# ArchDD/CPP-Raytracer-Rasterizer

Hardware: AMD Instinct MI355X
Metric: Mrays/s (primary+shadow) (higher is better)
Workload: dtype f32

## Files before the change

### cpp-raytracer-rasterizer_amd/capi/binned.cpp

```cpp
#include "capi.hpp"

namespace mirt {


int ensure_pairs(RtScratch &S, size_t cap)
{
    int r;
    if ((r = dev_realloc(&S.d_entries, cap)) || (r = dev_realloc(&S.d_pair_keys, cap)) || (r = dev_realloc(&S.d_pair_vals, cap)) ||
        (r = dev_realloc(&S.d_sorted_keys, cap)) || (r = dev_realloc(&S.d_tmp_vals, cap))) { S.cap_entries = 0; return r; }
    S.cap_entries = (uint32_t)cap;
    return MIRT_OK;
}

constexpr uint32_t BIN_MAX_KEYS = BUCKET_SORT_MAX_BUCKETS * 1024u - 1u;

void poll_pair_count(RtScratch &S)
{
    if (S.count_pending && hipEventQuery(S.ev_count) == hipSuccess) {
        S.known_pairs = *S.h_count; S.have_known = true; S.count_pending = false;
    }
    (void)hipGetLastError();
}

int bin_pass(RtScratch &S, BinSet bs, const OriginRow *cam_tab, const OriginRow *light_tab, uint32_t *counter, uint32_t *bin_off,
             bool fresh, uint32_t *npairs, bool may_guess = false)
{
    int rc;
    poll_pair_count(S);
    if (!fresh && may_guess && S.have_known && S.known_pairs > S.cap_used) fresh = true;
    const bool guess = fresh && may_guess && S.have_known;
    if (!S.d_entries || !S.cap_entries) {
        static const size_t initial = [] { const long v = env_int("MIRT_BIN_INITIAL_PAIRS", 0); return v > 0 ? (size_t)v : (size_t)1 << 20; }();
        if ((rc = ensure_pairs(S, initial))) return rc;
    }
    if (bs.nbins > BIN_MAX_KEYS) return fail(MIRT_ERR_INVALID_ARGUMENT, "binning: %u sort keys exceed the %u the bucket sort holds", bs.nbins, BIN_MAX_KEYS);
    bs.chunk_tris = 256;
    const dim3 bin_grid((unsigned)std::min<long long>((long long)((g.n + bs.chunk_tris - 1) / bs.chunk_tris) * bs.nframes, (long long)g.cu_count * 8));
    bs.counters = counter;
    const uint32_t nbuckets = bucket_sort_buckets(bs.nbins);
    if (nbuckets + 1 > S.cap_buckets) {
        S.cap_buckets = 0;
        if ((rc = dev_realloc(&S.d_bucket, (size_t)3 * (nbuckets + 1)))) return rc;
        HIP_TRY(hipMemsetAsync(S.d_bucket, 0, sizeof(uint32_t) * 3 * (nbuckets + 1), g.stream));
        S.cap_buckets = nbuckets + 1;
        S.bucket_dirty = false;
    }
    uint32_t *bcnt = S.d_bucket, *bbase = S.d_bucket + S.cap_buckets, *bcur = S.d_bucket + 2 * (size_t)S.cap_buckets;
    bs.bucket_cnt = bcnt; bs.nbuckets = nbuckets; bs.bucket_shift = bucket_sort_shift(bs.nbins);
    const size_t bin_lds = (size_t)nbuckets * sizeof(uint32_t);
    {
        static const bool once = [] {
            (void)hipFuncSetAttribute(reinterpret_cast<const void *>(&k_bin_pairs<512>), hipFuncAttributeMaxDynamicSharedMemorySize, 48 * 1024);
            (void)hipFuncSetAttribute(reinterpret_cast<const void *>(&k_bin_pairs<256>), hipFuncAttributeMaxDynamicSharedMemorySize, 48 * 1024);
            return true; }();
        (void)once;
    }
    static const int bin_wg_env = (int)env_int("MIRT_BIN_WG", 0);
    const int bin_wg = (bin_wg_env == 256 || bin_wg_env == 512) ? bin_wg_env : ((g.n < 400000 && g.in_flight >= 3) ? 256 : 512);
    if (guess) {
        const size_t want = (size_t)S.known_pairs + S.known_pairs / 2 + 4096;
        if (want > S.cap_entries) {
            HIP_TRY(hipStreamSynchronize(g.stream));
            if ((rc = ensure_pairs(S, want + want / 4))) return rc;
        }
    }
    bool publish_count = false;
    for (int attempt = 0; attempt < 2; attempt++) {
        static const uint32_t test_cap = [] { const long v = env_int("MIRT_TEST_PAIR_CAP", 0); return v > 0 ? (uint32_t)v : 0u; }();
        S.cap_used = (guess && test_cap && test_cap < S.cap_entries) ? test_cap : S.cap_entries;
        BinPairs pairs = { S.d_pair_keys, S.d_pair_vals, S.cap_used };
        bs.entries = S.d_entries; bs.cap_entries = S.cap_used;
        if (attempt) HIP_TRY(hipMemsetAsync(counter, 0, 4, g.stream));
        if (attempt || S.bucket_dirty) HIP_TRY(hipMemsetAsync(S.d_bucket, 0, sizeof(uint32_t) * 3 * (size_t)S.cap_buckets, g.stream));
        S.bucket_dirty = true;
        if (bin_wg == 256) hipLaunchKernelGGL(k_bin_pairs<256>, bin_grid, dim3(256), bin_lds, g.stream, g.d_tris, cam_tab, light_tab, g.n, bs, pairs);
        else hipLaunchKernelGGL(k_bin_pairs<512>, bin_grid, dim3(512), bin_lds, g.stream, g.d_tris, cam_tab, light_tab, g.n, bs, pairs);
        if (!fresh) break;
        if (guess) {
            if (!S.h_count) {
                HIP_TRY(hipHostMalloc(reinterpret_cast<void **>(&S.h_count), 64, hipHostMallocDefault));
                HIP_TRY(hipEventCreateWithFlags(&S.ev_count, hipEventDisableTiming));
            }
            if (!S.count_pending) publish_count = true;
            *npairs = S.known_pairs;
            break;
        }
        uint32_t total = 0;
        HIP_TRY(hipStreamSynchronize(g.stream));
        HIP_TRY(hipMemcpy(&total, counter, 4, hipMemcpyDeviceToHost));
        *npairs = total;
        S.known_pairs = total; S.have_known = true;
        S.count_pending = false;
        if (total <= S.cap_entries) break;
        if (attempt == 1) return fail(MIRT_ERR_HIP, "binning produced %u pairs twice with room for %u", total, S.cap_entries);
        if ((rc = ensure_pairs(S, (size_t)total + total / 8 + 4096))) return rc;
    }
#ifdef MIRT_BIN_STATS
    if (fresh) {
        uint32_t c[16];
        (void)hipMemcpy(c, counter, 64, hipMemcpyDeviceToHost);
        fprintf(stderr, "[mirt bin stats] flattened tests=%u max per work item=%u direct items=%u | huge: box valid=%u no box=%u (camera frame %u)\n", c[8], c[9], c[10], c[11], c[12], c[14]);
        fprintf(stderr, "[mirt bin stats] tris=%d frames=%d  pairs=%u  bins=%u | large items walked=%u level-1 rounds=%u level-2 steps=%u pairs=%u max steps/item=%u items>100 steps=%u\n",
                g.n, bs.nframes, *npairs, bs.nbins, c[2], c[3], c[4], c[5], c[6], c[7]);
        (void)hipMemset(counter + 2, 0, 56);
    }
#endif
    uint32_t *count_out = nullptr;
    if (publish_count) HIP_TRY(hipHostGetDevicePointer(reinterpret_cast<void **>(&count_out), S.h_count, 0));
    HIP_TRY(bucket_sort_pairs(S.d_pair_keys, S.d_pair_vals, counter, S.cap_used, *npairs, bs.nbins, S.d_sorted_keys, S.d_tmp_vals,
                              bcnt, bbase, bcur, bin_off, S.d_entries, g.cu_count, g.stream, count_out));
    S.bucket_dirty = false;
    if (publish_count) S.count_event_due = true;
    return MIRT_OK;
}

uint64_t light_key_of(const float *origins, int nlights)
{
    uint64_t key = 0xcbf29ce484222325ull ^ g.scene_version;
    auto mix = [&](const void *p, size_t nb) { const unsigned char *b = (const unsigned char *)p; for (size_t i = 0; i < nb; i++) { key ^= b[i]; key *= 0x100000001b3ull; } };
    mix(origins + 3, sizeof(float) * 3 * nlights); mix(&nlights, 4); mix(&g.n, 4);
    return key;
}

bool shell_range(const float *pos, double *dn, double *df)
{
    double n2 = 0.0, f2 = 0.0;
    for (int c = 0; c < 3; c++) {
        const double p = pos[c], lo = g.bbox_lo[c], hi = g.bbox_hi[c];
        const double near = p < lo ? lo - p : (p > hi ? p - hi : 0.0), far = std::max(std::fabs(p - lo), std::fabs(p - hi));
        n2 += near * near; f2 += far * far;
    }
    *dn = std::sqrt(n2); *df = std::sqrt(f2);
    return std::isfinite(*dn) && std::isfinite(*df) && *df > *dn;
}

void fill_light_frames(BinFrameDesc *frames, const RtFrame &f, int nlights, int cube_bins, int shells, uint32_t base_bins)
{
    memset(frames, 0, sizeof(BinFrameDesc) * 6 * nlights);
    for (int k = 0; k < nlights; k++) {
        double dn = 0.0, df = 0.0;
        const bool okr = shell_range(f.lpos[k], &dn, &df);
        for (int face = 0; face < 6; face++) {
            BinFrameDesc &d = frames[k * 6 + face];
            const int ax = face >> 1;
            d.P0[ax] = (face & 1) ? -1.0f : 1.0f;
            d.Pu[(ax + 1) % 3] = 1.0f;
            d.Pv[(ax + 2) % 3] = 1.0f;
            d.rw[ax] = d.P0[ax]; d.ru[(ax + 1) % 3] = 1.0f; d.rv[(ax + 2) % 3] = 1.0f;
            memcpy(d.S, f.lpos[k], 12);
            d.dmax = 2.0f;
            d.ulo = -1.0f; d.vlo = -1.0f; d.du = 2.0f / (float)cube_bins; d.dv = 2.0f / (float)cube_bins;
            d.pad_lo = -3.814697265625e-06f; d.pad_hi = 3.814697265625e-06f;
            d.nbu = cube_bins; d.nbv = cube_bins; d.j0 = 0; d.j1 = cube_bins;
            d.base = base_bins; d.tab = 1 + k;
            d.nshell = shells;
            d.shell_d0 = (float)dn;
            d.shell_iw = okr ? (float)(shells / (df - dn)) : 0.0f;
            base_bins += (uint32_t)(cube_bins * cube_bins);
        }
    }
}

int light_shells_for(int nlights, int cube_bins, uint32_t keys_in_front)
{
    static const int env = (int)env_int("MIRT_LIGHT_SHELLS", 0);
    const long long bins = 6ll * cube_bins * cube_bins * std::max(nlights, 1);
    int ns = (env >= 1 && env <= 64) ? env : 16;
    while (ns > 1 && bins * ns + keys_in_front + 64 > (long long)BIN_MAX_KEYS) ns >>= 1;
    return ns;
}

constexpr size_t LIGHT_COUNTER_BYTES = sizeof(uint32_t) * (128 + 6 * MIRT_MAX_LIGHTS);
int ensure_face_lists(RtScratch &S, int nlights)
{
    int rc;
    if (!S.d_bin_counters) {
        HIP_TRY(hipMalloc(reinterpret_cast<void **>(&S.d_bin_counters), LIGHT_COUNTER_BYTES));
        HIP_TRY(hipMemsetAsync(S.d_bin_counters, 0, LIGHT_COUNTER_BYTES, g.stream));
        S.d_face_counts = S.d_bin_counters + 128;
    }
    const size_t want = (size_t)6 * (size_t)nlights * (size_t)g.n;
    if (want > S.cap_face_sel) {
        HIP_TRY(hipStreamSynchronize(g.stream));
        S.cap_face_sel = 0;
        if ((rc = dev_realloc(&S.d_face_sel, want))) return rc;
        S.cap_face_sel = want;
    }
    return MIRT_OK;
}

int light_cache_ensure(RtScratch &S, const RtFrame &f, const float *origins, int nlights, int cube_bins)
{
    int rc;
    LightCache &C = g.lc;
    const uint64_t key = light_key_of(origins, nlights);
    if (C.valid && C.key == key && C.cube_bins == cube_bins) return MIRT_OK;
    C.valid = false;
    for (int o = 0; o < g.in_flight; o++)
        if (o != g.si) {
            HIP_TRY(hipEventRecord(g.streams[o].ev_order, g.streams[o].stream));
            HIP_TRY(hipStreamWaitEvent(g.stream, g.streams[o].ev_order, 0));
        }
    const int shells = light_shells_for(nlights, cube_bins, 0u);
    const uint32_t per_light = 6u * (uint32_t)(cube_bins * cube_bins) * (uint32_t)shells, nkeys = per_light * (uint32_t)nlights;
    if ((size_t)nlights * g.n > C.cap_tab) {
        C.cap_tab = 0;
        if ((rc = dev_realloc(&C.d_light_tab, (size_t)nlights * g.n))) return rc;
        C.cap_tab = (size_t)nlights * g.n;
    }
    if (nkeys + 1 > C.cap_bins) {
        C.cap_bins = 0;
        if ((rc = dev_realloc(&C.d_off, (size_t)nkeys + 1))) return rc;
        C.cap_bins = nkeys + 1;
    }
    if (!C.d_frames) HIP_TRY(hipMalloc(reinterpret_cast<void **>(&C.d_frames), sizeof(BinFrameDesc) * 6 * MIRT_MAX_LIGHTS));
    if (!C.d_origins) HIP_TRY(hipMalloc(reinterpret_cast<void **>(&C.d_origins), sizeof(float) * 3 * (1 + MIRT_MAX_LIGHTS)));
    if (!C.d_counter) { HIP_TRY(hipMalloc(reinterpret_cast<void **>(&C.d_counter), 512)); HIP_TRY(hipMemsetAsync(C.d_counter, 0, 512, g.stream)); }
    C.nbins = nkeys;
    C.nrows = 0;
    C.shells = shells;
    if (nlights > 0) {
        BinFrameDesc frames[6 * MIRT_MAX_LIGHTS];
        fill_light_frames(frames, f, nlights, cube_bins, shells, 0u);
        HIP_TRY(upload_small(C.d_frames, frames, sizeof(BinFrameDesc) * 6 * nlights, g.stream));
        HIP_TRY(upload_small(C.d_origins, origins, sizeof(float) * 3 * (1 + nlights), g.stream));
        if ((rc = ensure_face_lists(S, nlights))) return rc;
        HIP_TRY(hipMemsetAsync(S.d_face_counts, 0, sizeof(uint32_t) * 6 * nlights, g.stream));
        HIP_TRY(hipMemsetAsync(C.d_counter, 0, 512, g.stream));
        S.count_event_due = false;
        hipLaunchKernelGGL(k_select_faces, dim3((unsigned)std::min<long long>(((long long)g.n + 1023) / 1024, (long long)g.cu_count), nlights), dim3(1024), 0, g.stream,
                           g.d_tris, g.n, C.d_origins, C.d_frames, C.d_light_tab, S.d_face_sel, (uint32_t)g.n, S.d_face_counts);
        BinSet bs;
        memset(&bs, 0, sizeof bs);
        bs.frames = C.d_frames; bs.nframes = 6 * nlights; bs.nbins = nkeys; bs.bin_off = C.d_off;
        bs.face_lists = S.d_face_sel; bs.face_counts = S.d_face_counts; bs.face_stride = (uint32_t)g.n;
        uint32_t npairs = 0;
        if ((rc = bin_pass(S, bs, nullptr, C.d_light_tab, C.d_counter, C.d_off, true, &npairs))) return rc;
        S.count_event_due = false;
        if (npairs > C.cap_rows) {
            C.cap_rows = 0;
            if ((rc = dev_realloc(&C.d_rows, (size_t)npairs + npairs / 8 + 1024))) return rc;
            if ((rc = dev_realloc(&C.d_row_tri, (size_t)npairs + npairs / 8 + 1024))) return rc;
            C.cap_rows = npairs + npairs / 8 + 1024;
        }
        C.nrows = npairs;
        if (npairs)
            hipLaunchKernelGGL(k_expand_light_rows, dim3((unsigned)std::min<uint32_t>((npairs + 255) / 256, 4096u)), dim3(256), 0, g.stream,
                               C.d_off, S.d_entries, nlights, per_light, C.d_light_tab, g.n, C.d_rows, (const uint32_t *)nullptr, 0u, C.d_row_tri);
        HIP_TRY(hipGetLastError());
        S.bin_key_valid = false;
        S.last_bin_mode = -1;
    } else {
        HIP_TRY(hipMemsetAsync(C.d_off, 0, 4, g.stream));
    }
    if (g.in_flight > 1) {
        HIP_TRY(hipEventRecord(g.cur().ev_order, g.stream));
        for (int o = 0; o < g.in_flight; o++)
            if (o != g.si) HIP_TRY(hipStreamWaitEvent(g.streams[o].stream, g.cur().ev_order, 0));
    }
    C.key = key;
    C.cube_bins = cube_bins;
    C.valid = true;
    return MIRT_OK;
}

int camera_shells_for(long long tiles)
{
    static const int shells_env = (int)env_int("MIRT_CAM_SHELLS", 0);
    int ns = (int)std::min<long long>(8, std::max<long long>(1, (4ll << 20) / std::max<long long>(tiles, 1)));
    if (shells_env >= 1 && shells_env <= 64) ns = shells_env;
    while (ns > 1 && tiles * ns + 64 > (long long)BIN_MAX_KEYS) ns >>= 1;
    return ns;
}

bool frame_fits_binning(int W, int H)
{
    const long long tiles = (long long)((W + BIN_TILE - 1) / BIN_TILE) * ((H + BIN_TILE - 1) / BIN_TILE);
    return tiles + 64 <= (long long)BIN_MAX_KEYS;
}

constexpr int LIGHT_STABLE_FRAMES = 4;


int transient_light_pass(RtScratch &L, const RtFrame &f, const float *origins, int nlights, int cube_bins, int tshells, uint32_t per_light, uint64_t lkey, bool *kept,
                         unsigned long long *zero_hits )
{
    int rc;
    *kept = false;
    uint64_t key = 0xcbf29ce484222325ull ^ g.scene_version;
    {
        auto mix = [&](const void *p, size_t nb) { const unsigned char *b = (const unsigned char *)p; for (size_t i = 0; i < nb; i++) { key ^= b[i]; key *= 0x100000001b3ull; } };
        mix(&lkey, 8); mix(&cube_bins, 4); mix(&tshells, 4); mix(&g.n, 4); mix(&nlights, 4);
    }
    poll_pair_count(L);
    bool fresh = !L.bin_key_valid || L.bin_key != key;
    const bool may_guess = L.last_bin_mode == nlights;
    if (!fresh && L.have_known && L.known_pairs > L.cap_used) fresh = true;
    static const bool reuse_off = env_int("MIRT_BIN_REUSE", 1) == 0;
    if (!fresh && !reuse_off) { *kept = true; return MIRT_OK; }
    if ((rc = ensure_face_lists(L, nlights))) return rc;
    if (nlights > L.light_tab_lights || L.light_tab_n != g.n) {
        HIP_TRY(hipStreamSynchronize(g.stream));
        L.light_tab_lights = 0;
        if ((rc = dev_realloc(&L.d_light_tab, (size_t)nlights * g.n))) return rc;
        L.light_tab_lights = nlights;
        L.light_tab_n = g.n;
    }
    const uint32_t nkeys = per_light * (uint32_t)nlights;
    if (nkeys + 1 > L.cap_bins) {
        HIP_TRY(hipStreamSynchronize(g.stream));
        L.cap_bins = 0;
        if ((rc = dev_realloc(&L.d_bin_off, (size_t)nkeys + 1))) return rc;
        L.cap_bins = nkeys + 1;
    }
    if (!L.d_frames) HIP_TRY(hipMalloc(reinterpret_cast<void **>(&L.d_frames), sizeof(BinFrameDesc) * (6 * MIRT_MAX_LIGHTS) + sizeof(float) * 3 * (1 + MIRT_MAX_LIGHTS)));
    struct { BinFrameDesc frames[6 * MIRT_MAX_LIGHTS]; float origins[3 * (1 + MIRT_MAX_LIGHTS)]; } up;
    static_assert(sizeof(BinFrameDesc) % 4 == 0, "descriptors are uploaded as words");
    fill_light_frames(up.frames, f, nlights, cube_bins, tshells, 0u);
    float *d_origins = reinterpret_cast<float *>(L.d_frames + 6 * nlights);
    memcpy(reinterpret_cast<char *>(up.frames + 6 * nlights), origins, sizeof(float) * 3 * (1 + nlights));
    const ZeroJob zj = { L.d_bin_counters, (int)(LIGHT_COUNTER_BYTES / 4), reinterpret_cast<uint32_t *>(zero_hits), zero_hits ? 2 * HIT_SHARDS * HIT_SHARD_STRIDE : 0 };
    HIP_TRY(upload_small(L.d_frames, &up, sizeof(BinFrameDesc) * 6 * nlights + sizeof(float) * 3 * (1 + nlights), g.stream, &zj));
    hipLaunchKernelGGL(k_select_faces, dim3((unsigned)std::min<long long>(((long long)g.n + 1023) / 1024, (long long)g.cu_count), nlights), dim3(1024), 0, g.stream,
                       g.d_tris, g.n, d_origins, L.d_frames, L.d_light_tab, L.d_face_sel, (uint32_t)g.n, L.d_face_counts);
    BinSet bs;
    memset(&bs, 0, sizeof bs);
    bs.frames = L.d_frames; bs.nframes = 6 * nlights; bs.nbins = nkeys; bs.bin_off = L.d_bin_off;
    bs.face_lists = L.d_face_sel; bs.face_counts = L.d_face_counts; bs.face_stride = (uint32_t)g.n;
    if ((rc = bin_pass(L, bs, nullptr, L.d_light_tab, L.d_bin_counters, L.d_bin_off, true, &L.bin_entries, may_guess))) return rc;
    L.last_bin_mode = nlights;
    L.bin_key = key;
    L.bin_key_valid = true;
    if (L.cap_light_rows < L.cap_entries) {
        HIP_TRY(hipStreamSynchronize(g.stream));
        L.cap_light_rows = 0;
        if ((rc = dev_realloc(&L.d_light_rows, (size_t)L.cap_entries))) return rc;
        L.cap_light_rows = L.cap_entries;
    }
    const uint32_t expect = std::max<uint32_t>(L.bin_entries, 1u);
    hipLaunchKernelGGL(k_expand_light_rows, dim3((unsigned)std::min<uint32_t>((expect + 255) / 256, 4096u)), dim3(256), 0, g.stream,
                       L.d_bin_off, L.d_entries, nlights, per_light, L.d_light_tab, g.n, L.d_light_rows, L.d_bin_counters, L.cap_used, (uint32_t *)nullptr);
    return MIRT_OK;
}

int binned_pass(const RtFrame &f, const mirt_view *view, RtScratch &S, RtScratch &L, const float *origins, int nlights, int y0, int y1, BinnedPass *bp)
{
    int rc;
    g.stats.mode_used = MIRT_RT_BINNED;
    g.stats_sel_count = nullptr;
    static const int cube_override = (int)env_int("MIRT_CUBE_BINS", 0);
    int fine_bins = g.n < 2000 ? CUBE_BINS_MIN : (g.n < 20000 ? 2 * CUBE_BINS_MIN : 4 * CUBE_BINS_MIN);
    const bool fixed_grid = cube_override == 64 || cube_override == 128 || cube_override == 256;
    if (fixed_grid) fine_bins = cube_override;
    while (fine_bins > CUBE_BINS_MIN && 6ll * fine_bins * fine_bins * nlights * 4 > (long long)BIN_MAX_KEYS) fine_bins /= 2;

    const uint64_t lkey = light_key_of(origins, nlights);
    if (g.lc.track_key == lkey) g.lc.stable++;
    else { g.lc.track_key = lkey; g.lc.stable = 0; }
    const bool cached = g.lc.valid && g.lc.key == lkey && g.lc.cube_bins == fine_bins;
    const bool transient = nlights > 0 && !fixed_grid && !cached && g.lc.stable < LIGHT_STABLE_FRAMES;

    k_begin(MIRT_K_BIN);
    if (!transient && (rc = light_cache_ensure(L, f, origins, nlights, fine_bins))) return rc;
    const int cube_bins = transient ? CUBE_BINS_MIN : fine_bins;

    BinSet bs;
    memset(&bs, 0, sizeof bs);
    bs.frame0 = make_camera_frame(view, y0, y1, g.aa);
    bs.frames = nullptr; bs.nframes = 1;
    const int band_tile_rows = bs.frame0.j1 - bs.frame0.j0;
    const uint32_t key_shift_tiles = (uint32_t)bs.frame0.j0 * (uint32_t)bs.frame0.nbu;
    bs.frame0.base = 0u - key_shift_tiles;
    {
        const int ns = camera_shells_for((long long)bs.frame0.nbu * band_tile_rows);
        double dn = 0.0, df = 0.0;
        const bool okr = shell_range(view->pos, &dn, &df);
        bs.frame0.nshell = okr ? ns : 1;
        bs.frame0.shell_d0 = (float)dn;
        bs.frame0.shell_iw = okr ? (float)(ns / (df - dn)) : 0.0f;
    }
    const uint32_t cam_keys = (uint32_t)bs.frame0.nbu * (uint32_t)band_tile_rows * (uint32_t)bs.frame0.nshell;
    const int tshells = transient ? light_shells_for(nlights, cube_bins, 0u) : 1;
    const uint32_t per_light = 6u * (uint32_t)(cube_bins * cube_bins) * (uint32_t)tshells;
    bs.nbins = cam_keys;
    if (bs.nbins + 1 > S.cap_bins) {
        const size_t cap = (size_t)bs.nbins + 1;
        HIP_TRY(hipStreamSynchronize(g.stream));
        if ((rc = dev_realloc(&S.d_bin_off, cap))) { S.cap_bins = 0; return rc; }
        S.cap_bins = (uint32_t)cap;
        S.bin_key_valid = false;
    }
    if (!S.d_bin_counters) { HIP_TRY(hipMalloc(reinterpret_cast<void **>(&S.d_bin_counters), 512)); HIP_TRY(hipMemsetAsync(S.d_bin_counters, 0, 512, g.stream)); }
    if (S.sel_n != g.n) {
        HIP_TRY(hipStreamSynchronize(g.stream));
        S.sel_n = 0;
        if ((rc = dev_realloc(&S.d_sel, (size_t)g.n))) return rc;
        S.sel_n = g.n;
        S.bin_key_valid = false;
    }
    bs.bin_off = S.d_bin_off;

    uint64_t key = 0xcbf29ce484222325ull ^ g.scene_version;
    {
        auto mix = [&](const void *p, size_t nb) { const unsigned char *b = (const unsigned char *)p; for (size_t i = 0; i < nb; i++) { key ^= b[i]; key *= 0x100000001b3ull; } };
        mix(view, sizeof *view); mix(&y0, 4); mix(&y1, 4); mix(&g.n, 4); mix(&g.aa, 4);
    }
    const int bin_mode = 0;
    StreamState &ss = g.cur();
    ss.hits_clean[ss.hits_tog] = false;
    if (!S.d_frames) HIP_TRY(hipMalloc(reinterpret_cast<void **>(&S.d_frames), sizeof(BinFrameDesc) * (1 + 6 * MIRT_MAX_LIGHTS)));
    poll_pair_count(S);
    bool fresh = !S.bin_key_valid || S.bin_key != key;
    const bool may_guess = S.last_bin_mode == bin_mode;
    if (!fresh && S.have_known && S.known_pairs > S.cap_used) fresh = true;
    static const bool reuse_off = env_int("MIRT_BIN_REUSE", 1) == 0;
    const bool reuse = !fresh && !reuse_off;
    const uint32_t pairs_x = (uint32_t)((bs.frame0.nbu + 1) / 2);
    uint32_t group_rows[ORDER_GROUPS] = { 0 };
    for (int j = bs.frame0.j0; j < bs.frame0.j1; j++) group_rows[((uint32_t)j >> ORDER_STRIPE_SHIFT) & (ORDER_GROUPS - 1)]++;
    const uint32_t order_seg = pairs_x * *std::max_element(group_rows, group_rows + ORDER_GROUPS);
    const uint32_t *cam_off = S.d_bin_off - (size_t)key_shift_tiles * (size_t)bs.frame0.nshell;
    bool lights_kept = false, forked = false;
    if (transient) {
        static const bool side_off = env_int("MIRT_LIGHT_SIDE_STREAM", 1) == 0;
        hipStream_t main_stream = g.stream;
        forked = !reuse && !side_off;
        if (forked) {
            HIP_TRY(hipEventRecord(ss.ev_fork, main_stream));
            HIP_TRY(hipStreamWaitEvent(ss.aux, ss.ev_fork, 0));
            g.stream = ss.aux;
        }
        rc = transient_light_pass(L, f, origins, nlights, cube_bins, tshells, per_light, lkey, &lights_kept, reuse ? g.d_hits : nullptr);
        g.stream = main_stream;
        if (rc) return rc;
        if (forked) HIP_TRY(hipEventRecord(ss.ev_join, ss.aux));
    }
    if (reuse) {
        if (!(transient && !lights_kept)) HIP_TRY(hipMemsetAsync(g.d_hits, 0, HIT_BYTES, g.stream));
        g.stats.bins_reused = 1;
    } else {
        S.sel_parity ^= 1;
        SelectOut so;
        memset(&so, 0, sizeof so);
        so.cam_tab = S.d_cam_tab; so.sel = S.d_sel;
        so.sel_count = S.d_bin_counters + SEL_COUNT0 + S.sel_parity; so.sel_count_next = S.d_bin_counters + SEL_COUNT0 + (S.sel_parity ^ 1);
        so.zero_hits = g.d_hits; so.zero_counter = S.d_bin_counters;
        if ((rc = hist_prepare(S, bs.frame0, &so))) return rc;
        const unsigned sel_grid = (unsigned)std::min<long long>(((long long)g.n + 1023) / 1024, (long long)g.cu_count);
        hipLaunchKernelGGL(k_prep_select, dim3(sel_grid), dim3(1024), 0, g.stream, g.d_tris, g.n, bs.frame0, so);
        if ((rc = hist_publish(S))) return rc;
        bs.sel = S.d_sel; bs.sel_count = so.sel_count;
        g.stats_sel_count = so.sel_count;
        if ((rc = bin_pass(S, bs, S.d_cam_tab, nullptr, S.d_bin_counters, S.d_bin_off, true, &S.bin_entries, may_guess))) return rc;
        S.last_bin_mode = bin_mode;
        S.bin_key = key;
        S.bin_key_valid = true;
        if ((size_t)order_seg > S.cap_order) {
            HIP_TRY(hipStreamSynchronize(g.stream));
            S.cap_order = 0;
            if ((rc = dev_realloc(&S.d_order, (size_t)ORDER_GROUPS * ORDER_CLASSES * order_seg))) return rc;
            S.cap_order = order_seg;
        }
        hipLaunchKernelGGL(k_tile_order, dim3((pairs_x + 63) / 64, (unsigned)(bs.frame0.j1 - bs.frame0.j0)), dim3(64), 0, g.stream, cam_off, bs.frame0.nshell,
                           bs.frame0.nbu, bs.frame0.j0, bs.frame0.j1, S.d_bin_counters, S.cap_used, S.d_order, order_seg);
    }
    if (forked) HIP_TRY(hipStreamWaitEvent(g.stream, ss.ev_join, 0));
    k_end(MIRT_K_BIN);

    bp->cam_off = cam_off;
    bp->tiles_x = bs.frame0.nbu;
    bp->cam_shells = bs.frame0.nshell;
    bp->order_seg = order_seg;
    bp->transient = transient;
    bp->cube_bins = cube_bins;
    bp->light_shells = transient ? tshells : g.lc.shells;
    return MIRT_OK;
}

int hist_only_pass(const mirt_view *view)
{
    int rc;
    g.stream = g.cur().stream;
    RtScratch &S = g.cur().rt;
    if (S.cam_tab_n != g.n) {
        S.cam_tab_n = 0;
        if ((rc = dev_realloc(&S.d_cam_tab, (size_t)g.n))) return rc;
        S.cam_tab_n = g.n;
    }
    if (S.sel_n != g.n) {
        HIP_TRY(hipStreamSynchronize(g.stream));
        S.sel_n = 0;
        if ((rc = dev_realloc(&S.d_sel, (size_t)g.n))) return rc;
        S.sel_n = g.n;
    }
    if (!S.d_bin_counters) { HIP_TRY(hipMalloc(reinterpret_cast<void **>(&S.d_bin_counters), 512)); HIP_TRY(hipMemsetAsync(S.d_bin_counters, 0, 512, g.stream)); }
    S.bin_key_valid = false;
    const BinFrameDesc fr = make_camera_frame(view, 0, 0, g.aa);
    SelectOut so;
    memset(&so, 0, sizeof so);
    so.cam_tab = S.d_cam_tab; so.sel = S.d_sel;
    so.sel_count = S.d_bin_counters + HIST_SEL_COUNT; so.sel_count_next = S.d_bin_counters + HIST_SEL_COUNT + 1;
    if ((rc = hist_prepare(S, fr, &so))) return rc;
    if (!g.hist_armed) return MIRT_OK;
    HIP_TRY(hipMemsetAsync(so.sel_count, 0, 4, g.stream));
    const unsigned sel_grid = (unsigned)std::min<long long>(((long long)g.n + 1023) / 1024, (long long)g.cu_count);
    if (sel_grid) hipLaunchKernelGGL(k_prep_select, dim3(sel_grid), dim3(1024), 0, g.stream, g.d_tris, g.n, fr, so);
    HIP_TRY(hipGetLastError());
    return hist_publish(S);
}

int binned_trace(const RtFrame &f, RtScratch &S, RtScratch &L, const BinnedPass &bp)
{
    const bool transient = bp.transient;
    RtTraceFrame tf;
    memset(&tf, 0, sizeof tf);
    tf.f = f;
    tf.f.cam_tab = S.d_cam_tab;
    tf.f.light_tab = transient ? L.d_light_tab : g.lc.d_light_tab;
    tf.f.unsafe = nullptr;
    tf.cam_off = bp.cam_off;
    tf.cam_entries = S.d_entries;
    tf.sel = S.d_sel; tf.sel_count = S.d_bin_counters + SEL_COUNT0 + S.sel_parity;
    static const int lazy_env = (int)env_int("MIRT_LAZY_GEO", -1);
    tf.lazy_geo = lazy_env >= 0 ? (lazy_env != 0) : (g.n >= 400000);
    tf.geo = g.d_geo;
    tf.shade = g.d_shade;
    tf.light_off = transient ? L.d_bin_off : g.lc.d_off;
    tf.light_rows = transient ? L.d_light_rows : g.lc.d_rows;
    tf.light_tri = transient ? L.d_entries : g.lc.d_row_tri;
    tf.light_frames = transient ? L.d_frames : g.lc.d_frames;
    tf.tiles_x = bp.tiles_x;
    tf.cube_bins = bp.cube_bins;
    tf.cam_shells = bp.cam_shells;
    tf.light_shells = bp.light_shells;
    tf.pair_count = S.d_bin_counters;
    tf.pair_cap = S.cap_used;
    tf.light_pair_count = transient ? L.d_bin_counters : nullptr;
    tf.light_pair_cap = L.cap_used;
    tf.order = S.d_order; tf.order_count = S.d_bin_counters + 16; tf.order_seg = bp.order_seg;
    const dim3 tgrid(ORDER_GROUPS * bp.order_seg);
    const size_t lds = rt_trace_lds_bytes(1);
    k_begin(MIRT_K_TRACE);
    g.pending_counted = g.profiling;
    if (f.aa > 1) {
        if (g.profiling) hipLaunchKernelGGL((k_rt_trace2<true, true>), tgrid, dim3(64), lds, g.stream, tf);
        else hipLaunchKernelGGL((k_rt_trace2<true, false>), tgrid, dim3(64), lds, g.stream, tf);
    } else {
        static const int waves5_env = (int)env_int("MIRT_TR_WAVES5", -1);
        const bool waves5 = waves5_env >= 0 ? (waves5_env != 0) : (g.n >= 400000 || g.in_flight <= 2);
        if (g.profiling) hipLaunchKernelGGL((k_rt_trace2<false, true>), tgrid, dim3(64), lds, g.stream, tf);
        else if (waves5) hipLaunchKernelGGL((k_rt_trace2<false, false, 5>), tgrid, dim3(64), lds, g.stream, tf);
        else hipLaunchKernelGGL((k_rt_trace2<false, false>), tgrid, dim3(64), lds, g.stream, tf);
    }
    k_end(MIRT_K_TRACE);
    HIP_TRY(hipGetLastError());
    for (RtScratch *P : { &S, &L })
        if (P->count_event_due) {
            P->count_event_due = false;
            HIP_TRY(hipEventRecord(P->ev_count, g.stream));
            P->count_pending = true;
        }
    return MIRT_OK;
}

}
```

### cpp-raytracer-rasterizer_amd/capi/capi.hpp

```cpp
#pragma once

#include "../csrc/bin_sort.hpp"
#include "../csrc/comm.hpp"
#include "../csrc/cull.hpp"
#include "../csrc/dof.hpp"
#include "../csrc/rt_common.hpp"
#include "../csrc/raster_common.hpp"
#include "../csrc/rt_binned.hpp"
#include "../csrc/scan.hpp"
#include "env.hpp"

#include <cstdarg>
#include <cstdio>
#include <cstdlib>
#include <cstring>
#include <algorithm>
#include <cmath>
#include <vector>

#define MIRT_KERNEL __attribute__((global))

namespace mirt {

MIRT_KERNEL void k_prep_origin(const float *, int, const float *, v3, int, OriginRow *, OriginRow *, uint32_t *, unsigned long long *, uint32_t *);
template <int P> MIRT_KERNEL void k_rt_brute(const RtFrame);
template <int P> MIRT_KERNEL void k_rt_small(const RtFrame, int);
MIRT_KERNEL void k_rt_wave(const RtFrame);
struct RtTileFrame {
    RtFrame f;
    BinFrameDesc cam;
    int tiles_x, tiles_y;
    unsigned long long *clear_hits;
    float4 *tables;
};
MIRT_KERNEL void k_tile_tables(const RtTileFrame);
template <int TW, bool AA> MIRT_KERNEL void k_rt_tile2(const RtTileFrame);
template <int WG> MIRT_KERNEL void k_bin_pairs(const float *, const OriginRow *, const OriginRow *, int, BinSet, BinPairs);
struct TilePairRec { uint32_t tile, beg, nA, nB; };
constexpr int ORDER_CLASSES = 8, ORDER_GROUPS = 8;
struct RtTraceFrame {
    RtFrame f;
    const uint32_t *cam_off;
    const uint32_t *cam_entries;
    const GeoRow *geo;
    const ShadeRow *shade;
    const uint32_t *light_off;
    const LightRow *light_rows;
    const uint32_t *light_tri;
    const BinFrameDesc *light_frames;
    int tiles_x;
    int cube_bins;
    int cam_shells;
    int light_shells;
    const uint32_t *pair_count;
    uint32_t pair_cap;
    const TilePairRec *order;
    const uint32_t *order_count;
    uint32_t order_seg;
    const uint32_t *sel;
    const uint32_t *sel_count;
    int lazy_geo;
    const uint32_t *light_pair_count;
    uint32_t light_pair_cap;
};
template <bool AA, bool STATS, int WAVES = 4> MIRT_KERNEL void k_rt_trace2(const RtTraceFrame);
MIRT_KERNEL void k_prep_select(const float *, int, const BinFrameDesc, const SelectOut);
MIRT_KERNEL void k_select_faces(const float *, int, const float *, const BinFrameDesc *, OriginRow *, uint32_t *, uint32_t, uint32_t *);
MIRT_KERNEL void k_tile_order(const uint32_t *, int, int, int, int, uint32_t *, uint32_t, TilePairRec *, uint32_t);
MIRT_KERNEL void k_geo_table(const float *, int, GeoRow *, ShadeRow *);
MIRT_KERNEL void k_expand_light_rows(const uint32_t *, const uint32_t *, int, uint32_t, const OriginRow *, int, LightRow *, const uint32_t *, uint32_t, uint32_t *);
MIRT_KERNEL void k_cull(const float *, int, const CullParams, uint8_t *);
size_t rt_trace_lds_bytes(int waves);
int launch_raster(RasterFrame &f, RasterScratch &s, uint64_t scene_version, hipStream_t stream, hipEvent_t *ev, bool *ev_used);

extern char g_err[512];
int fail(int code, const char *fmt, ...);

#define HIP_TRY(expr)                                                                          \
    do {                                                                                       \
        hipError_t e_ = (expr);                                                                \
        if (e_ != hipSuccess)                                                                  \
            return fail(MIRT_ERR_HIP, "%s failed: %s (%s:%d)", #expr, hipGetErrorString(e_), __FILE__, __LINE__); \
    } while (0)

enum { EV_CALL0 = 0, EV_CALL1 = 1, EV_K0 = 2, EV_COUNT = 2 + 2 * 8 };
constexpr int MAX_FLIGHT = 4;
constexpr int SEL_COUNT0 = 80;
constexpr int HIST_SEL_COUNT = 82;
constexpr int HIST_RING = 4;
constexpr int HIST_SLOTS = HIST_RING + 1;
constexpr size_t HIT_BYTES = sizeof(unsigned long long) * HIT_SHARDS * HIT_SHARD_STRIDE;

struct RtScratch {
    OriginRow *d_cam_tab = nullptr;
    OriginRow *d_light_tab = nullptr;
    int cam_tab_n = 0, light_tab_n = 0, light_tab_lights = 0;
    float *d_origins = nullptr;
    uint32_t *d_flags = nullptr;
    BinFrameDesc *d_frames = nullptr;
    uint32_t *d_bin_off = nullptr, *d_bin_counters = nullptr;
    uint32_t *d_entries = nullptr;
    uint32_t *d_pair_keys = nullptr, *d_pair_vals = nullptr, *d_sorted_keys = nullptr;
    uint32_t *d_tmp_vals = nullptr;
    uint32_t *d_bucket = nullptr;
    uint32_t cap_buckets = 0;
    bool bucket_dirty = false;
    uint32_t *h_count = nullptr;
    hipEvent_t ev_count = nullptr;
    bool count_pending = false;
    bool count_event_due = false;
    bool have_known = false;
    uint32_t known_pairs = 0;
    uint32_t cap_bins = 0, cap_entries = 0;
    uint32_t cap_used = 0;
    uint64_t bin_key = 0;
    uint32_t bin_entries = 0;
    bool bin_key_valid = false;
    LightRow *d_light_rows = nullptr;
    uint32_t cap_light_rows = 0;
    TilePairRec *d_order = nullptr;
    uint32_t cap_order = 0;
    int last_bin_mode = -1;
    uint32_t *d_sel = nullptr;
    int sel_n = 0;
    int sel_parity = 0;
    uint32_t *d_face_sel = nullptr;
    size_t cap_face_sel = 0;
    uint32_t *d_face_counts = nullptr;
    uint32_t *d_hist = nullptr;
    uint32_t *h_hist = nullptr;
    hipEvent_t ev_hist[HIST_SLOTS] = {};
    uint64_t hist_key[HIST_SLOTS] = {};
    uint64_t hist_seq[HIST_SLOTS] = {};
    int hist_rows[HIST_SLOTS] = {}, hist_shift[HIST_SLOTS] = {};
    int hist_next = 0;

    void forget_scene() { bin_key_valid = false; have_known = false; count_pending = false; }
    void release();
};

struct LightCache {
    bool valid = false;
    uint64_t key = 0;
    int cube_bins = 0;
    uint64_t track_key = 0;
    int stable = 0;
    OriginRow *d_light_tab = nullptr;
    size_t cap_tab = 0;
    BinFrameDesc *d_frames = nullptr;
    uint32_t *d_off = nullptr;
    uint32_t cap_bins = 0, nbins = 0;
    LightRow *d_rows = nullptr;
    uint32_t *d_row_tri = nullptr;
    uint32_t cap_rows = 0, nrows = 0;
    int shells = 1;
    float *d_origins = nullptr;
    uint32_t *d_counter = nullptr;

    void release();
};

struct DofPlanes {
    float *rgb = nullptr, *fd = nullptr;
    uint32_t *xrgb = nullptr;
    int32_t *index = nullptr;
    float *zinv = nullptr;
    size_t cap_px = 0;

    int ensure(size_t px);
    void release();
};

struct StreamState {
    hipStream_t stream = nullptr;
    hipEvent_t ev_order = nullptr;
    hipStream_t aux = nullptr;
    hipEvent_t ev_fork = nullptr, ev_join = nullptr;
    hipEvent_t ev[EV_COUNT] = {};
    bool ev_used[8] = {};
    bool call_timed = false;
    RtScratch rt;
    RtScratch rt_lt;
    unsigned long long *d_hits[2] = {};
    bool hits_clean[2] = {};
    int hits_tog = 0;
    float4 *d_tile_tab = nullptr;
    DofPlanes dof;
    void *d_async = nullptr;
    RasterScratch raster;
    uint64_t culled_ver = 0;
    hipEvent_t ev_cull_read = nullptr;
    uint32_t cull_read_src = 0;

    int create();
    void release();
};

struct Ctx {
    bool init = false;
    bool profiling = false;
    int device = -1;
    int cu_count = 256;
    StreamState streams[MAX_FLIGHT];
    hipStream_t stream = nullptr;
    int in_flight = 1;
    uint64_t frame_no = 0;
    int si = 0;
    int ev_cur = 0;
    StreamState &cur() { return streams[si]; }

    int n = 0;
    float *d_tris = nullptr;
    uint8_t *d_culled = nullptr;
    int culled_latest = 0;
    uint64_t cull_calls = 0;
    GeoRow *d_geo = nullptr;
    ShadeRow *d_shade = nullptr;
    float bbox_lo[3] = { 0, 0, 0 }, bbox_hi[3] = { 0, 0, 0 };
    LightCache lc;
    unsigned long long *d_hits = nullptr;
    bool scene_finite = true;
    uint64_t scene_version = 0;
    uint64_t cull_version = 0;
    int soft_samples = 1;
    int aa = 1;
    int dof_k = 0;
    float dof_focal = 0.0f;
    int soft_npos = 0;
    float soft_pos[MIRT_MAX_LIGHTS * 3] = {};

    struct HostSurface { char *host = nullptr; char *dev = nullptr; size_t bytes = 0; } surf[4];

    void *d_xrgb = nullptr, *d_rgb = nullptr, *d_index = nullptr, *d_zinv = nullptr, *d_pos = nullptr;
    size_t cap_px = 0;
    size_t async_cap_px = 0;

    Comm *comm = nullptr;
    hipStream_t comm_stream = nullptr;
    hipEvent_t ev_rendered = nullptr, ev_sent[2] = { nullptr, nullptr };
    char *d_band[2] = { nullptr, nullptr };
    size_t band_bytes[2] = { 0, 0 };
    int band_slot = 0;
    int strip_rows = 0;
    bool want_hist = false;
    uint64_t shard_calls = 0;
    bool hist_call = false;
    uint64_t hist_seq = 0;
    bool in_sharded = false;
    bool hist_armed = false;

    mirt_stats stats = {};
    bool stats_pending = false;
    bool raster_since_sync = false;
    hipStream_t stats_stream = nullptr;
    uint64_t pending_primary = 0;
    int pending_nlights = 0;
    bool pending_is_rt = false;
    bool pending_counted = false;
    bool pending_empty = false;
    const uint32_t *stats_sel_count = nullptr;
};

extern Ctx g;

int need_init();
int dev_realloc_bytes(void **p, size_t bytes);
template <typename T> int dev_realloc(T **p, size_t count) { return dev_realloc_bytes(reinterpret_cast<void **>(p), count * sizeof(T)); }
int check_frame_args(const mirt_view *view, const mirt_light *lights, int nlights, const float *indirect, const void *xrgb, int pitch_bytes,
                     bool need_scene = false, int y0 = 0, int y1 = 0);
hipError_t sync_all();
int next_si();
void call_begin();
void call_end();
inline void k_begin(int k) { if (g.profiling) { (void)hipEventRecord(g.cur().ev[EV_K0 + 2 * k], g.stream); g.cur().ev_used[k] = true; } }
inline void k_end(int k) { if (g.profiling) (void)hipEventRecord(g.cur().ev[EV_K0 + 2 * k + 1], g.stream); }
struct ZeroJob { uint32_t *a; int na; uint32_t *b; int nb; };
hipError_t upload_small(void *dst, const void *src, size_t bytes, hipStream_t stream, const ZeroJob *zero = nullptr);
void hist_out(uint32_t *hist, uint32_t *host_copy, hipStream_t stream);

int rt_enqueue(const mirt_view *view, const mirt_light *lights, int nlights, const float *indirect, int mode,
               int y0, int y1, int row_origin, void *d_xrgb, int pitch_bytes, void *d_rgb, void *d_index, void *d_fd = nullptr,
               void *d_dist = nullptr, void *d_pos = nullptr);
BinFrameDesc make_camera_frame(const mirt_view *view, int y0, int y1, int aa);
bool frame_fits_binning(int W, int H);
struct BinnedPass {
    const uint32_t *cam_off;
    int tiles_x, cam_shells;
    uint32_t order_seg;
    bool transient;
    int cube_bins, light_shells;
};
int binned_pass(const RtFrame &f, const mirt_view *view, RtScratch &S, RtScratch &L, const float *origins, int nlights, int y0, int y1, BinnedPass *bp);
int binned_trace(const RtFrame &f, RtScratch &S, RtScratch &L, const BinnedPass &bp);
bool rt_bins_whole_frame(const mirt_view *view, const mirt_light *lights, int nlights, int mode);
int hist_only_pass(const mirt_view *view);

int raster_enqueue(const mirt_view *view, const mirt_light *lights, int nlights, const float *indirect,
                   int y0, int y1, int row_origin, void *d_xrgb, int pitch_bytes, void *d_rgb, void *d_zinv,
                   void *d_index, void *d_fd = nullptr);
int cull_copy_wait_readers(int dst, hipStream_t st);

int hist_prepare(RtScratch &S, const BinFrameDesc &cam, SelectOut *so);
int hist_publish(RtScratch &S);
const uint32_t *hist_lookup(uint64_t max_key, int *rows, int *shift);
void current_bounds(int world, int W, int H, std::vector<int> &bounds);
unsigned part_tile_weight();
int plan_out(int world, int root, int width, int height, int nviews, int strip_rows, const int *bounds, uint64_t *root_offset,
             uint64_t *band_offset, uint64_t *bytes, int32_t *peer, int max_pieces);
int render_sharded(const mirt_view *views, int nviews, int root, void *d_frames, int pitch_bytes, bool raster,
                   const mirt_light *lights, int nlights, const float *indirect, int mode);

struct HostPlane { void *host; void **staging; size_t bpp; };
int ensure_staging(size_t px, const HostPlane *planes, int nplanes);
char *registered_alias(const void *host, size_t pitch, int H);
bool host_direct();
int copy_plane_interior(void *dst, int dst_pitch, const void *src, int src_pitch, int W, int H);
int async_plane(size_t px, void **plane);
int async_target(const mirt_view *view, const mirt_light *lights, int nlights, const float *indirect, uint32_t *out_xrgb, int pitch_bytes, char **alias);
int dof_resolve(const DofPlanes &D, const mirt_view *view, int y0, int y1, int row_origin, int ry0, int ry1, void *d_xrgb, int pitch_bytes,
                void *user_rgb, void *user_index, void *user_zinv, bool clear_border);

template <class Render>
int render_with_dof(const mirt_view *view, const mirt_light *lights, int nlights, const float *indirect, int y0, int y1, int row_origin,
                    void *d_xrgb, int pitch_bytes, void *user_rgb, void *user_index, void *user_zinv, bool clear_border, Render render)
{
    int rc;
    if ((rc = check_frame_args(view, lights, nlights, indirect, d_xrgb, pitch_bytes, false, y0, y1))) return rc;
    const int W = view->width, H = view->height, K = g.dof_k;
    const int zlo = (int)std::ceil((float)K / -2.0f), zhi = (int)std::ceil((float)K / 2.0f);
    const int reach = std::max(-zlo, zhi - 1) + 1;
    const int ry0 = std::max(0, y0 - reach), ry1 = std::min(H, y1 + reach);
    DofPlanes &D = g.streams[next_si()].dof;
    if ((rc = D.ensure((size_t)W * (size_t)(ry1 - ry0)))) return rc;
    const ptrdiff_t shift = (ptrdiff_t)ry0 * W;
    if ((rc = render(ry0, ry1, (void *)D.xrgb, (void *)(D.rgb - 3 * shift), (void *)(D.fd - shift), user_index ? (void *)(D.index - shift) : nullptr,
                     user_zinv ? (void *)(D.zinv - shift) : nullptr))) return rc;
    return dof_resolve(D, view, y0, y1, row_origin, ry0, ry1, d_xrgb, pitch_bytes, user_rgb, user_index, user_zinv, clear_border);
}

template <int N, class Render>
int deliver_host(const mirt_view *view, const mirt_light *lights, int nlights, const float *indirect, uint32_t *out_xrgb, int pitch_bytes,
                 bool writes_every_word, const HostPlane (&planes)[N], Render render)
{
    int rc;
    if ((rc = check_frame_args(view, lights, nlights, indirect, out_xrgb, pitch_bytes))) return rc;
    const int W = view->width, H = view->height;
    const size_t px = (size_t)W * H;
    if ((rc = ensure_staging(px, planes, N))) return rc;
    char *alias = registered_alias(out_xrgb, (size_t)pitch_bytes, H);
    const bool direct = alias && host_direct();
    void *dev[N];
    for (int i = 0; i < N; i++) dev[i] = planes[i].host ? *planes[i].staging : nullptr;
    if ((rc = render(direct ? (void *)alias : g.d_xrgb, direct ? pitch_bytes : W * 4, dev))) return rc;
    if (!direct) {
        if (writes_every_word) HIP_TRY(hipMemcpy2DAsync(out_xrgb, pitch_bytes, g.d_xrgb, (size_t)W * 4, (size_t)W * 4, H, hipMemcpyDeviceToHost, g.stream));
        else if ((rc = copy_plane_interior(out_xrgb, pitch_bytes, g.d_xrgb, W * 4, W, H))) return rc;
    }
    for (int i = 0; i < N; i++)
        if (planes[i].host) HIP_TRY(hipMemcpyAsync(planes[i].host, dev[i], px * planes[i].bpp, hipMemcpyDeviceToHost, g.stream));
    HIP_TRY(hipStreamSynchronize(g.stream));
    return MIRT_OK;
}

template <class Render>
int deliver_async(const mirt_view *view, const mirt_light *lights, int nlights, const float *indirect, uint32_t *out_xrgb, int pitch_bytes,
                  bool writes_every_word, Render render)
{
    int rc;
    char *alias = nullptr;
    if ((rc = async_target(view, lights, nlights, indirect, out_xrgb, pitch_bytes, &alias))) return rc;
    const int W = view->width, H = view->height;
    if (host_direct()) return render((void *)alias, pitch_bytes);
    void *plane = nullptr;
    if ((rc = async_plane((size_t)W * H, &plane))) return rc;
    if ((rc = render(plane, W * 4))) return rc;
    if (!writes_every_word) return copy_plane_interior(out_xrgb, pitch_bytes, plane, W * 4, W, H);
    HIP_TRY(hipMemcpy2DAsync(out_xrgb, pitch_bytes, plane, (size_t)W * 4, (size_t)W * 4, H, hipMemcpyDeviceToHost, g.stream));
    return MIRT_OK;
}

}
```

### cpp-raytracer-rasterizer_amd/csrc/bin_bucket_sort.hip

```cpp
#include "bin_sort.hpp"

#include <algorithm>
#include <cstdlib>

namespace mirt {

constexpr int BS_PER_THREAD = 16;
constexpr int BS_CHUNK = 256 * BS_PER_THREAD;
constexpr int BS_LOCAL_PER_THREAD = 16;
constexpr int BS_MAX_SHIFT = 12;
constexpr int BS_MAX_BUCKET_KEYS = 1 << BS_MAX_SHIFT;

__device__ __forceinline__ uint32_t bs_block_scan(uint32_t v, uint32_t *s_wave , uint32_t *total)
{
    const int lane = threadIdx.x & 63, wave = threadIdx.x >> 6;
    uint32_t incl = v;
#pragma unroll
    for (int d = 1; d < 64; d <<= 1) {
        const uint32_t o = __shfl_up(incl, d);
        if (lane >= d) incl += o;
    }
    __syncthreads();
    if (lane == 63) s_wave[wave] = incl;
    __syncthreads();
    uint32_t off = 0, all = 0;
#pragma unroll
    for (int w = 0; w < 4; w++) { if (w < wave) off += s_wave[w]; all += s_wave[w]; }
    *total = all;
    return off + incl - v;
}

__global__ __launch_bounds__(256) void k_bs_scatter(const uint32_t *__restrict__ keys, const uint32_t *__restrict__ vals,
                                                    const uint32_t *__restrict__ total_ptr, uint32_t cap, uint32_t nbuckets, int shift,
                                                    const uint32_t *__restrict__ bucket_cnt, uint32_t *__restrict__ bucket_base,
                                                    uint32_t *__restrict__ cursor, uint32_t *__restrict__ out_keys, uint32_t *__restrict__ out_vals,
                                                    uint32_t *__restrict__ count_out)
{
    extern __shared__ uint32_t s_dyn[];
    __shared__ uint32_t s_wave[4];
    if (count_out && blockIdx.x == 0 && threadIdx.x == 0) *count_out = *total_ptr;
    if (*total_ptr > cap) return;
    uint32_t *s_base = s_dyn, *s_cnt = s_dyn + nbuckets;
    uint32_t carry = 0;
    for (uint32_t b0 = 0; b0 < nbuckets; b0 += 256) {
        const uint32_t b = b0 + threadIdx.x;
        const uint32_t c = b < nbuckets ? bucket_cnt[b] : 0u;
        uint32_t all;
        const uint32_t excl = carry + bs_block_scan(c, s_wave, &all);
        if (b < nbuckets) { s_base[b] = excl; if (blockIdx.x == 0) bucket_base[b] = excl; }
        carry += all;
    }
    if (blockIdx.x == 0 && threadIdx.x == 0) bucket_base[nbuckets] = carry;
    const uint32_t total = min(*total_ptr, cap);
    for (uint32_t base = blockIdx.x * BS_CHUNK; base < total; base += gridDim.x * BS_CHUNK) {
        for (uint32_t b = threadIdx.x; b < nbuckets; b += 256) s_cnt[b] = 0u;
        __syncthreads();
        uint32_t k[BS_PER_THREAD], v[BS_PER_THREAD], rank[BS_PER_THREAD];
#pragma unroll
        for (int j = 0; j < BS_PER_THREAD; j++) {
            const uint32_t i = base + threadIdx.x + 256u * j;
            k[j] = 0xFFFFFFFFu; v[j] = 0u; rank[j] = 0u;
            if (i < total) { k[j] = keys[i]; v[j] = vals[i]; }
        }
#pragma unroll
        for (int j = 0; j < BS_PER_THREAD; j++)
            if (k[j] != 0xFFFFFFFFu) rank[j] = atomicAdd(&s_cnt[k[j] >> shift], 1u);
        __syncthreads();
        for (uint32_t b0 = threadIdx.x; b0 < nbuckets; b0 += 1024) {
            uint32_t c[4], at[4];
#pragma unroll
            for (int q = 0; q < 4; q++) { const uint32_t b = b0 + 256u * q; c[q] = b < nbuckets ? s_cnt[b] : 0u; at[q] = 0u; }
#pragma unroll
            for (int q = 0; q < 4; q++) if (c[q]) at[q] = atomicAdd(&cursor[b0 + 256u * q], c[q]);
#pragma unroll
            for (int q = 0; q < 4; q++) if (c[q]) s_cnt[b0 + 256u * q] = s_base[b0 + 256u * q] + at[q];
        }
        __syncthreads();
#pragma unroll
        for (int j = 0; j < BS_PER_THREAD; j++)
            if (k[j] != 0xFFFFFFFFu) {
                const uint32_t at = s_cnt[k[j] >> shift] + rank[j];
                out_keys[at] = k[j];
                out_vals[at] = v[j];
            }
        __syncthreads();
    }
}

__global__ __launch_bounds__(256) void k_bs_local(const uint32_t *__restrict__ keys, const uint32_t *__restrict__ vals,
                                                  const uint32_t *__restrict__ total_ptr, uint32_t cap,
                                                  const uint32_t *__restrict__ bucket_base, uint32_t nbins, int shift,
                                                  uint32_t *__restrict__ bucket_cnt, uint32_t *__restrict__ cursor,
                                                  uint32_t *__restrict__ bin_off, uint32_t *__restrict__ entries)
{
    __shared__ uint32_t s_cnt[BS_MAX_BUCKET_KEYS], s_wave[4];
    const uint32_t bucket = blockIdx.x;
    if (threadIdx.x == 0) { bucket_cnt[bucket] = 0u; cursor[bucket] = 0u; }
    if (*total_ptr > cap) return;
    const uint32_t beg = bucket_base[bucket], end = bucket_base[bucket + 1];
    const uint32_t nb = 1u << shift, mask = nb - 1u;
    for (uint32_t i = threadIdx.x; i < nb; i += 256) s_cnt[i] = 0u;
    __syncthreads();
    const bool small = end - beg <= 256u * BS_LOCAL_PER_THREAD;
    uint32_t lo[BS_LOCAL_PER_THREAD], v[BS_LOCAL_PER_THREAD], rank[BS_LOCAL_PER_THREAD];
    if (small) {
#pragma unroll
        for (int j = 0; j < BS_LOCAL_PER_THREAD; j++) {
            const uint32_t i = beg + threadIdx.x + 256u * j;
            lo[j] = 0xFFFFFFFFu; v[j] = 0u; rank[j] = 0u;
            if (i < end) { lo[j] = keys[i] & mask; v[j] = vals[i]; }
        }
#pragma unroll
        for (int j = 0; j < BS_LOCAL_PER_THREAD; j++)
            if (lo[j] != 0xFFFFFFFFu) rank[j] = atomicAdd(&s_cnt[lo[j]], 1u);
    } else {
        for (uint32_t i = beg + threadIdx.x; i < end; i += 256) atomicAdd(&s_cnt[keys[i] & mask], 1u);
    }
    __syncthreads();
    uint32_t carry = beg;
    for (uint32_t i0 = 0; i0 < nb; i0 += 256) {
        const uint32_t i = i0 + threadIdx.x;
        const uint32_t c = i < nb ? s_cnt[i] : 0u;
        uint32_t all;
        const uint32_t excl = carry + bs_block_scan(c, s_wave, &all);
        if (i < nb) {
            s_cnt[i] = excl;
            const uint32_t bin = (bucket << shift) + i;
            if (bin <= nbins) bin_off[bin] = excl;
        }
        carry += all;
    }
    __syncthreads();
    if (small) {
#pragma unroll
        for (int j = 0; j < BS_LOCAL_PER_THREAD; j++)
            if (lo[j] != 0xFFFFFFFFu) entries[s_cnt[lo[j]] + rank[j]] = v[j];
    } else {
        for (uint32_t i = beg + threadIdx.x; i < end; i += 256) {
            const uint32_t at = atomicAdd(&s_cnt[keys[i] & mask], 1u);
            entries[at] = vals[i];
        }
    }
}

int bucket_sort_shift(uint32_t nbins)
{
    int shift = 8;
    while (shift < BS_MAX_SHIFT && ((nbins + 1u + (1u << shift) - 1u) >> shift) > 1024u) shift++;
    while (shift > 4 && ((nbins + 1u + (1u << shift) - 1u) >> shift) < 512u) shift--;
    return shift;
}
uint32_t bucket_sort_buckets(uint32_t nbins) { const int s = bucket_sort_shift(nbins); return (nbins + 1u + (1u << s) - 1u) >> s; }

hipError_t bucket_sort_pairs(const uint32_t *keys, const uint32_t *vals, const uint32_t *total_ptr, uint32_t cap, uint32_t expected,
                             uint32_t nbins, uint32_t *tmp_keys, uint32_t *tmp_vals, uint32_t *bucket_cnt, uint32_t *bucket_base,
                             uint32_t *cursor, uint32_t *bin_off, uint32_t *entries, int cu_count, hipStream_t stream, uint32_t *count_out)
{
    const int shift = bucket_sort_shift(nbins);
    const uint32_t nbuckets = bucket_sort_buckets(nbins);
    const size_t lds = (size_t)nbuckets * 2 * sizeof(uint32_t);
    uint32_t chunks = (expected + BS_CHUNK - 1) / BS_CHUNK;
    if (chunks < 1) chunks = 1;
    const uint32_t wgs = std::min<uint32_t>(chunks, (uint32_t)cu_count * 2u);
    hipLaunchKernelGGL(k_bs_scatter, dim3(wgs), dim3(256), lds, stream, keys, vals, total_ptr, cap, nbuckets, shift, bucket_cnt, bucket_base,
                       cursor, tmp_keys, tmp_vals, count_out);
    hipLaunchKernelGGL(k_bs_local, dim3(nbuckets), dim3(256), 0, stream, tmp_keys, tmp_vals, total_ptr, cap, bucket_base, nbins, shift, bucket_cnt,
                       cursor, bin_off, entries);
    return hipGetLastError();
}

}
```

### cpp-raytracer-rasterizer_amd/csrc/rt_binned.hip

```cpp
#include "rt_binned.hpp"

#include <float.h>

namespace mirt {

constexpr int BIN_L0 = BIN_COARSE * BIN_COARSE;

struct BinItem {
    float A0[4], A1[4], A2[4], Bu[4], Bv[4];
    float lou, hiu, lov, hiv;
};

__device__ __forceinline__ float bcastf(float v, int lane) { return __builtin_bit_cast(float, __builtin_amdgcn_readlane(__builtin_bit_cast(int, v), lane)); }

__device__ __forceinline__ float corner(float s, float lo, float hi) { return fmaxf(s * lo, s * hi); }

__device__ __forceinline__ bool cell_may_hit(const BinItem &u, const float (&A)[4], float I, float J, float K)
{
    bool ok = true;
#pragma unroll
    for (int k = 0; k < 4; k++) ok = ok && (__builtin_fmaf(J, u.Bv[k], __builtin_fmaf(I, u.Bu[k], A[k])) >= 0.0f);
    return ok && (I + K >= u.lou) && (I <= u.hiu) && (J + K >= u.lov) && (J <= u.hiv);
}

struct BinLin { float a, bu, bv; };

__device__ __forceinline__ bool bin_triple_infeasible(const BinLin &f, const BinLin &g, const BinLin &h, float U, float V)
{
    const float f1 = g.bu * h.bv, f2 = g.bv * h.bu, g1 = h.bu * f.bv, g2 = h.bv * f.bu, h1 = f.bu * g.bv, h2 = f.bv * g.bu;
    float wf = f1 - f2, wg = g1 - g2, wh = h1 - h2;
    const bool pos = wf >= 0.0f && wg >= 0.0f && wh >= 0.0f, neg = wf <= 0.0f && wg <= 0.0f && wh <= 0.0f;
    if (!(pos || neg)) return false;
    if (neg) { wf = -wf; wg = -wg; wh = -wh; }
    if (!(wf + wg + wh > 0.0f)) return false;
    const float C = wf * f.a + wg * g.a + wh * h.a;
    const float slack = (fabsf(f1) + fabsf(f2)) * (fabsf(f.a) + fabsf(f.bu) * U + fabsf(f.bv) * V) +
                        (fabsf(g1) + fabsf(g2)) * (fabsf(g.a) + fabsf(g.bu) * U + fabsf(g.bv) * V) +
                        (fabsf(h1) + fabsf(h2)) * (fabsf(h.a) + fabsf(h.bu) * U + fabsf(h.bv) * V);
    return C < -9.5367431640625e-07f * slack;
}

__device__ __forceinline__ bool bin_jointly_empty(const BinLin (&G)[4], float u0, float u1, float v0, float v1)
{
    const float U = fmaxf(fabsf(u0), fabsf(u1)), V = fmaxf(fabsf(v0), fabsf(v1));
    const BinLin side[4] = { { -u0, 1.0f, 0.0f }, { u1, -1.0f, 0.0f }, { -v0, 0.0f, 1.0f }, { v1, 0.0f, -1.0f } };
    bool empty = false;
#pragma unroll
    for (int i = 0; i < 4; i++)
#pragma unroll
        for (int j = i + 1; j < 4; j++) {
#pragma unroll
            for (int k = j + 1; k < 4; k++) empty = empty || bin_triple_infeasible(G[i], G[j], G[k], U, V);
#pragma unroll
            for (int sd = 0; sd < 4; sd++) empty = empty || bin_triple_infeasible(G[i], G[j], side[sd], U, V);
        }
    return empty;
}

struct BinFrameGrid { int nbu, fj0, fj1, cells_x, cy0, ncell; uint32_t fbase, nshell; };

constexpr int BIN_PAIR_BUF = 4096;
constexpr int BIN_TESTS_PER_THREAD = 2;
constexpr int BIN_DIRECT_SIDE = 32;

struct BinLargeSink {
    uint32_t *s_keys, *s_vals;
    uint32_t *s_fill;
    uint32_t *s_valid;
    uint32_t *g_count;
    BinPairs out;
    uint32_t *bucket_cnt;
    int bucket_shift;
};

__device__ __forceinline__ void bin_walk_large(const BinItem &u, uint32_t utri, uint32_t ushell, const BinFrameGrid &gr, int lane,
                                               const BinLargeSink &sink, unsigned long long cells0)
{
#ifdef MIRT_BIN_STATS
    uint32_t dbg_steps = 0, dbg_pairs = 0, dbg_l1 = 0;
#endif
    for (int c0 = 0; c0 < gr.ncell; c0 += 64) {
        const int c = c0 + lane, cx = c % gr.cells_x, cy = gr.cy0 + c / gr.cells_x;
        unsigned long long m0;
        if (c0 == 0 && gr.ncell <= 64) m0 = cells0;
        else m0 = __ballot(c < gr.ncell && cell_may_hit(u, u.A0, (float)(cx * BIN_L0), (float)(cy * BIN_L0), (float)BIN_L0));
        while (m0) {
            const int l0 = __builtin_ctzll(m0);
            m0 &= m0 - 1ull;
            const int ucx = __builtin_amdgcn_readlane(cx, l0), ucy = __builtin_amdgcn_readlane(cy, l0);
            const int ci = ucx * BIN_L0 + (lane & 7) * BIN_COARSE, cj = ucy * BIN_L0 + (lane >> 3) * BIN_COARSE;
            const bool pass1 = ci < gr.nbu && cj + BIN_COARSE > gr.fj0 && cj < gr.fj1 && cell_may_hit(u, u.A1, (float)ci, (float)cj, (float)BIN_COARSE);
            unsigned long long m1 = __ballot(pass1);
#ifdef MIRT_BIN_STATS
            dbg_l1++;
#endif
            while (m1) {
                const int cl = __builtin_ctzll(m1);
                m1 &= m1 - 1ull;
                const int i = ucx * BIN_L0 + (cl & 7) * BIN_COARSE + (lane & 7);
                const int j = ucy * BIN_L0 + (cl >> 3) * BIN_COARSE + (lane >> 3);
                const bool pass2 = i < gr.nbu && j >= gr.fj0 && j < gr.fj1 && cell_may_hit(u, u.A2, (float)i, (float)j, 1.0f);
                const unsigned long long m2 = __ballot(pass2);
#ifdef MIRT_BIN_STATS
                dbg_steps++; dbg_pairs += (uint32_t)__popcll(m2);
#endif
                if (!m2) continue;
                const uint32_t np = (uint32_t)__popcll(m2), rank = (uint32_t)__popcll(m2 & ((1ull << lane) - 1ull));
                const uint32_t key = (gr.fbase + (uint32_t)j * gr.nbu + i) * gr.nshell + ushell;
                uint32_t at0 = 0;
                if (lane == 0) at0 = atomicAdd(sink.s_fill, np);
                at0 = (uint32_t)__builtin_amdgcn_readfirstlane((int)at0);
                if (at0 + np <= (uint32_t)BIN_PAIR_BUF) {
                    if (pass2) { sink.s_keys[at0 + rank] = key; sink.s_vals[at0 + rank] = utri; }
                } else {
                    if (lane == 0) {
                        if (at0 < (uint32_t)BIN_PAIR_BUF) *sink.s_valid = at0;
                        at0 = atomicAdd(sink.g_count, np);
                    }
                    at0 = (uint32_t)__builtin_amdgcn_readfirstlane((int)at0);
                    if (pass2 && at0 + rank < sink.out.cap) { sink.out.keys[at0 + rank] = key; sink.out.vals[at0 + rank] = utri; }
                    if (pass2 && sink.bucket_cnt) atomicAdd(&sink.bucket_cnt[key >> sink.bucket_shift], 1u);
                }
            }
        }
    }
#ifdef MIRT_BIN_STATS
    if (lane == 0) {
        uint32_t *c = sink.g_count;
        atomicAdd(&c[2], 1u); atomicAdd(&c[3], dbg_l1); atomicAdd(&c[4], dbg_steps); atomicAdd(&c[5], dbg_pairs);
        atomicMax(&c[6], dbg_steps);
        if (dbg_steps > 100) atomicAdd(&c[7], 1u);
    }
#endif
}

constexpr int SEL_WG = 1024;
constexpr int SEL_STAGE = 8192;

__global__ __launch_bounds__(SEL_WG) void k_prep_select(const float *__restrict__ tris15, int n, const BinFrameDesc fr, const SelectOut out)
{
    __shared__ uint32_t s_hist[SEL_HIST_MAX];
    __shared__ uint32_t s_sel[SEL_STAGE];
    __shared__ uint32_t s_fill, s_base;
    const int lane = threadIdx.x & 63;
    if (blockIdx.x == 0) {
        if (out.zero_hits)
            for (int g = threadIdx.x; g < HIT_SHARDS * HIT_SHARD_STRIDE; g += SEL_WG) out.zero_hits[g] = 0ull;
        if (out.zero_counter && (threadIdx.x == 0 || (threadIdx.x >= 16 && threadIdx.x < 80))) out.zero_counter[threadIdx.x] = 0u;
        if (threadIdx.x == 0) *out.sel_count_next = 0u;
        if (out.zero_faces && (int)threadIdx.x < out.zero_faces_n) out.zero_faces[threadIdx.x] = 0u;
    }
    if (out.hist && threadIdx.x < SEL_HIST_MAX) s_hist[threadIdx.x] = 0u;
    if (threadIdx.x == 0) s_fill = 0u;
    __syncthreads();
    const v3 S = V3(fr.S[0], fr.S[1], fr.S[2]);
    const int nchunks = (n + SEL_WG - 1) / SEL_WG;
    const int hist_rows = ((fr.nbv - 1) >> out.hist_shift) + 1;
    auto flush = [&]() {
        __syncthreads();
        const uint32_t staged = s_fill;
        if (threadIdx.x == 0 && staged) s_base = atomicAdd(out.sel_count, staged);
        __syncthreads();
        const uint32_t base = s_base;
        for (uint32_t i = threadIdx.x; i < staged; i += SEL_WG) out.sel[base + i] = s_sel[i];
        __syncthreads();
        if (threadIdx.x == 0) s_fill = 0u;
        __syncthreads();
    };
    for (int c = blockIdx.x; c < nchunks; c += gridDim.x) {
        if (s_fill + (uint32_t)SEL_WG > (uint32_t)SEL_STAGE) flush();
        const int i = c * SEL_WG + (int)threadIdx.x;
        bool keep = false;
        OriginRow r;
        if (i < n) {
            const float *t15 = tris15 + (size_t)15 * i;
            r = make_origin_row(t15, S);
            PreBox box;
            bool boxed;
            keep = frame_may_see(r, ld3(t15), ld3(t15 + 3), ld3(t15 + 6), fr, &box, &boxed);
            if (out.hist && boxed) {
                const float flo_u = fmaxf(ceilf(box.lou) - 1.0f, 0.0f), fhi_u = fminf(floorf(box.hiu), (float)(fr.nbu - 1));
                const float flo_v = fmaxf(ceilf(box.lov) - 1.0f, 0.0f), fhi_v = fminf(floorf(box.hiv), (float)(fr.nbv - 1));
                if (flo_u <= fhi_u && flo_v <= fhi_v) {
                    const uint32_t wi = (uint32_t)((int)fhi_u - (int)flo_u + 1);
                    const int ja = (int)flo_v, jb = (int)fhi_v;
                    for (int cr = ja >> out.hist_shift; cr <= (jb >> out.hist_shift) && cr < hist_rows; cr++) {
                        const int lo = max(ja, cr << out.hist_shift), hi = min(jb, ((cr + 1) << out.hist_shift) - 1);
                        atomicAdd(&s_hist[cr], wi * (uint32_t)(hi - lo + 1));
                    }
                }
            }
            if (keep) out.cam_tab[i] = r;
        }
        const unsigned long long m = __builtin_amdgcn_ballot_w64(keep);
        if (m) {
            uint32_t at0 = 0;
            if (lane == 0) at0 = atomicAdd(&s_fill, (uint32_t)__popcll(m));
            at0 = (uint32_t)__builtin_amdgcn_readfirstlane((int)at0);
            if (keep) s_sel[at0 + (uint32_t)__popcll(m & ((1ull << lane) - 1ull))] = (uint32_t)i;
        }
        __syncthreads();
    }
    flush();
    if (out.hist && threadIdx.x < SEL_HIST_MAX) {
        const uint32_t v = s_hist[threadIdx.x];
        if (v && (int)threadIdx.x < hist_rows) atomicAdd(&out.hist[threadIdx.x], v);
    }
}

constexpr int FACE_STAGE = 2048;
__global__ __launch_bounds__(SEL_WG) void k_select_faces(const float *__restrict__ tris15, int n, const float *__restrict__ origins ,
                                                        const BinFrameDesc *__restrict__ faces , OriginRow *__restrict__ light_tab,
                                                        uint32_t *__restrict__ lists, uint32_t stride, uint32_t *__restrict__ face_counts)
{
    __shared__ uint32_t s_sel[6][FACE_STAGE];
    __shared__ uint32_t s_fill[6], s_base[6];
    const int lane = threadIdx.x & 63, k = (int)blockIdx.y;
    if (threadIdx.x < 6) s_fill[threadIdx.x] = 0u;
    __syncthreads();
    const v3 S = ld3(origins + 3 * (1 + k));
    const int nchunks = (n + SEL_WG - 1) / SEL_WG;
    auto flush = [&]() {
        __syncthreads();
        if (threadIdx.x < 6 && s_fill[threadIdx.x]) s_base[threadIdx.x] = atomicAdd(&face_counts[k * 6 + (int)threadIdx.x], s_fill[threadIdx.x]);
        __syncthreads();
#pragma unroll
        for (int f = 0; f < 6; f++) {
            const uint32_t staged = s_fill[f], base = s_base[f];
            uint32_t *dst = lists + (size_t)(k * 6 + f) * stride + base;
            for (uint32_t i = threadIdx.x; i < staged; i += SEL_WG) dst[i] = s_sel[f][i];
        }
        __syncthreads();
        if (threadIdx.x < 6) s_fill[threadIdx.x] = 0u;
        __syncthreads();
    };
    for (int c = blockIdx.x; c < nchunks; c += gridDim.x) {
        uint32_t most = 0;
#pragma unroll
        for (int f = 0; f < 6; f++) most = max(most, s_fill[f]);
        if (most + (uint32_t)SEL_WG > (uint32_t)FACE_STAGE) flush();
        const int i = c * SEL_WG + (int)threadIdx.x;
        uint32_t keep = 0;
        if (i < n) {
            const float *t15 = tris15 + (size_t)15 * i;
            OriginRow r = make_origin_row(t15, S);
            const v3 va = ld3(t15), vb = ld3(t15 + 3), vc = ld3(t15 + 6);
            r.r2.w = origin_far(va, vb, vc, S);
            light_tab[(size_t)k * n + i] = r;
            for (int f = 0; f < 6; f++) {
                PreBox box;
                bool boxed;
                if (frame_may_see(r, va, vb, vc, faces[k * 6 + f], &box, &boxed)) keep |= 1u << f;
            }
        }
#pragma unroll
        for (int f = 0; f < 6; f++) {
            const unsigned long long m = __builtin_amdgcn_ballot_w64((keep >> f) & 1u);
            if (m) {
                uint32_t at0 = 0;
                if (lane == 0) at0 = atomicAdd(&s_fill[f], (uint32_t)__popcll(m));
                at0 = (uint32_t)__builtin_amdgcn_readfirstlane((int)at0);
                if ((keep >> f) & 1u) s_sel[f][at0 + (uint32_t)__popcll(m & ((1ull << lane) - 1ull))] = (uint32_t)i;
            }
        }
        __syncthreads();
    }
    flush();
}


template <int WG>
__global__ __launch_bounds__(WG) void k_bin_pairs(const float *__restrict__ tris15, const OriginRow *__restrict__ cam_tab,
                                                   const OriginRow *__restrict__ light_tab, int n, BinSet bs, BinPairs out)
{
    extern __shared__ uint32_t s_bucket[];
    __shared__ uint32_t s_keys[BIN_PAIR_BUF], s_vals[BIN_PAIR_BUF];
    __shared__ float4 s_A2[256], s_Bu[256], s_Bv[256], s_box[256];
    __shared__ uint32_t s_org[256];
    __shared__ uint32_t s_ni[256];
    __shared__ uint32_t s_tri[256];
    __shared__ uint32_t s_pre[257];
    __shared__ uint32_t s_wave[4];
    __shared__ uint32_t s_base, s_fill, s_valid;
    const int lane = threadIdx.x & 63, wave = threadIdx.x >> 6;
    const int chunk_tris = bs.chunk_tris;
    const int nchunks = (n + chunk_tris - 1) / chunk_tris;
    const bool listed = bs.sel != nullptr;
    const uint32_t nsel = listed ? min(*bs.sel_count, (uint32_t)n) : 0u;
    const int cam_chunk = (listed && nsel < 32768u) ? 64 : chunk_tris;
    const int ncam = listed ? (int)((nsel + (uint32_t)cam_chunk - 1u) / (uint32_t)cam_chunk) : 0;
    const int nrest = listed ? bs.nframes - 1 : bs.nframes;
    const bool faces_listed = bs.face_lists != nullptr;
    __shared__ uint32_t s_first[MAX_BIN_FRAMES + 1];
    if (faces_listed) {
        if (threadIdx.x == 0) {
            uint32_t run = 0;
            for (int ff = 0; ff < nrest; ff++) { s_first[ff] = run; run += (min(bs.face_counts[ff], (uint32_t)n) + (uint32_t)chunk_tris - 1u) / (uint32_t)chunk_tris; }
            s_first[nrest] = run;
        }
        __syncthreads();
    }
    const int nwork = ncam + (faces_listed ? (int)s_first[nrest] : nchunks * nrest);
    if (threadIdx.x == 0) { s_fill = 0u; s_valid = (uint32_t)BIN_PAIR_BUF; }
    if (bs.bucket_cnt)
        for (uint32_t b = threadIdx.x; b < bs.nbuckets; b += WG) s_bucket[b] = 0u;

    auto flush = [&]() {
        __syncthreads();
        const uint32_t staged = min(s_fill, s_valid);
        if (threadIdx.x == 0 && staged) s_base = atomicAdd(&bs.counters[0], staged);
        __syncthreads();
        const uint32_t base = s_base;
        for (uint32_t i = threadIdx.x; i < staged; i += WG) {
            const uint32_t at = base + i;
            if (at < out.cap) { out.keys[at] = s_keys[i]; out.vals[at] = s_vals[i]; }
            if (bs.bucket_cnt) atomicAdd(&s_bucket[s_keys[i] >> bs.bucket_shift], 1u);
        }
        __syncthreads();
        if (bs.bucket_cnt && staged)
            for (uint32_t b = threadIdx.x; b < bs.nbuckets; b += WG) {
                const uint32_t c = s_bucket[b];
                if (c) { atomicAdd(&bs.bucket_cnt[b], c); s_bucket[b] = 0u; }
            }
        if (threadIdx.x == 0) { s_fill = 0u; s_valid = (uint32_t)BIN_PAIR_BUF; }
        __syncthreads();
    };

#ifdef MIRT_BIN_STAMPS
    long long st_setup = 0, st_prefix = 0, st_rounds = 0, st_huge = 0, st_flush = 0, st_t;
    const long long st_begin = __builtin_amdgcn_s_memtime();
    int st_nrounds = 0;
#define STAMP(acc) { const long long now_ = __builtin_amdgcn_s_memtime(); acc += now_ - st_t; st_t = now_; }
#else
#define STAMP(acc)
#endif
    for (int w = blockIdx.x; w < nwork; w += gridDim.x) {
#ifdef MIRT_BIN_STAMPS
        st_t = __builtin_amdgcn_s_memtime();
#endif
        int chunk, frame;
        const uint32_t *list = nullptr;
        uint32_t nhere = (uint32_t)n;
        const bool from_cam_list = w < ncam;
        if (from_cam_list) { chunk = w; frame = 0; list = bs.sel; nhere = nsel; }
        else if (faces_listed) {
            const uint32_t w2 = (uint32_t)(w - ncam);
            int lo = 0, hi = nrest;
            while (hi - lo > 1) { const int mid = (lo + hi) >> 1; if (s_first[mid] <= w2) lo = mid; else hi = mid; }
            chunk = (int)(w2 - s_first[lo]);
            frame = lo + (listed ? 1 : 0);
            list = bs.face_lists + (size_t)lo * bs.face_stride;
            nhere = min(bs.face_counts[lo], (uint32_t)n);
        } else { const int w2 = w - ncam; chunk = w2 / nrest; frame = w2 - chunk * nrest + (listed ? 1 : 0); }
        const int item_tris = from_cam_list ? cam_chunk : chunk_tris;
        const uint32_t slot = (uint32_t)chunk * (uint32_t)item_tris + threadIdx.x;
        const uint32_t tri = ((int)threadIdx.x < item_tris && slot < nhere) ? (list ? list[slot] : slot) : 0xFFFFFFFFu;
        const BinFrameDesc fr = bs.frames ? bs.frames[frame] : bs.frame0;
        BinFrameGrid gr;
        gr.nbu = fr.nbu; gr.fj0 = fr.j0; gr.fj1 = fr.j1; gr.fbase = fr.base; gr.nshell = (uint32_t)max(fr.nshell, 1);
        gr.cells_x = (gr.nbu + BIN_L0 - 1) / BIN_L0; gr.cy0 = gr.fj0 / BIN_L0;
        gr.ncell = gr.cells_x * ((gr.fj1 + BIN_L0 - 1) / BIN_L0 - gr.cy0);
        const int nbu = gr.nbu, fj0 = gr.fj0, fj1 = gr.fj1;
        BinItem it;
        memset(&it, 0, sizeof it);
        int kind = 0;
#ifdef MIRT_BIN_STATS
        int dbg_state = 0;
#endif
        int i_lo = 0, i_hi = -1, j_lo = 0, j_hi = -1;
        unsigned long long cells = 0;
        uint32_t shell = 0;
        if (tri < (uint32_t)n && fj1 > fj0) {
            const OriginRow &row = (fr.tab == 0) ? cam_tab[tri] : light_tab[(size_t)(fr.tab - 1) * n + tri];
            shell = bin_shell_of(fr, row.r1.w);
            TriBinFns t = make_bin_fns(row, fr);
            add_bbox(t, tris15 + (size_t)15 * tri, fr);
#ifdef MIRT_BIN_STATS
            dbg_state = t.bstate == BOX_VALID ? 0 : (t.bstate == BOX_NONE ? 1 : 2);
#endif
            const float T = 1.6940658945086007e-21f;
            const bool both = fabsf(t.nb) < T || !(t.nb == t.nb);
            const float sgn = t.nb < 0.0f ? -1.0f : 1.0f;
            const EdgeFn *fn[4] = { &t.n, &t.p, &t.q, &t.s };
            const float inf = __builtin_huge_valf();
#pragma unroll
            for (int k = 0; k < 4; k++) {
                const float su = sgn * fn[k]->cu, sv = sgn * fn[k]->cv;
                const float base = sgn * fn[k]->c0 + fn[k]->m + su * fr.ulo + sv * fr.vlo;
                it.Bu[k] = both ? 0.0f : su * fr.du;
                it.Bv[k] = both ? 0.0f : sv * fr.dv;
                it.A0[k] = both ? inf : base + corner(su, fr.pad_lo, (float)BIN_L0 * fr.du + fr.pad_hi) + corner(sv, fr.pad_lo, (float)BIN_L0 * fr.dv + fr.pad_hi);
                it.A1[k] = both ? inf : base + corner(su, fr.pad_lo, (float)BIN_COARSE * fr.du + fr.pad_hi) + corner(sv, fr.pad_lo, (float)BIN_COARSE * fr.dv + fr.pad_hi);
                it.A2[k] = both ? inf : base + corner(su, fr.pad_lo, fr.du + fr.pad_hi) + corner(sv, fr.pad_lo, fr.dv + fr.pad_hi);
            }
            if (t.bstate == BOX_VALID) {
                it.lou = (t.bu0 - fr.ulo - fr.pad_hi) / fr.du; it.hiu = (t.bu1 - fr.ulo - fr.pad_lo) / fr.du;
                it.lov = (t.bv0 - fr.vlo - fr.pad_hi) / fr.dv; it.hiv = (t.bv1 - fr.vlo - fr.pad_lo) / fr.dv;
                it.lou -= 3.814697265625e-06f * (1.0f + fabsf(it.lou)); it.hiu += 3.814697265625e-06f * (1.0f + fabsf(it.hiu));
                it.lov -= 3.814697265625e-06f * (1.0f + fabsf(it.lov)); it.hiv += 3.814697265625e-06f * (1.0f + fabsf(it.hiv));
            } else if (t.bstate == BOX_EMPTY) {
                it.lou = it.lov = inf; it.hiu = it.hiv = -inf;
            } else {
                it.lou = it.lov = -inf; it.hiu = it.hiv = inf;
            }
            const float flo_u = fmaxf(ceilf(it.lou) - 1.0f, 0.0f), fhi_u = fminf(floorf(it.hiu), (float)(nbu - 1));
            const float flo_v = fmaxf(ceilf(it.lov) - 1.0f, (float)fj0), fhi_v = fminf(floorf(it.hiv), (float)(fj1 - 1));
            if (flo_u <= fhi_u && flo_v <= fhi_v) {
                i_lo = (int)flo_u; i_hi = (int)fhi_u; j_lo = (int)flo_v; j_hi = (int)fhi_v;
                kind = (i_hi - i_lo < BIN_DIRECT_SIDE && j_hi - j_lo < BIN_DIRECT_SIDE) ? 1 : 2;
            }
            if (kind == 2) {
                for (int c = 0; c < gr.ncell && c < 64; c++) {
                    const int cx = c % gr.cells_x, cy = gr.cy0 + c / gr.cells_x;
                    if (cell_may_hit(it, it.A0, (float)(cx * BIN_L0), (float)(cy * BIN_L0), (float)BIN_L0)) cells |= 1ull << c;
                }
                if (gr.ncell > 64) cells = ~0ull;
                if (!cells) kind = 0;
                if (kind == 2 && !both) {
                    BinLin G[4];
#pragma unroll
                    for (int k = 0; k < 4; k++) { G[k].a = sgn * fn[k]->c0 + fn[k]->m; G[k].bu = sgn * fn[k]->cu; G[k].bv = sgn * fn[k]->cv; }
                    const float u0 = fr.ulo + fr.pad_lo, u1 = fr.ulo + (float)nbu * fr.du + fr.pad_hi;
                    const float v0 = fr.vlo + (float)fj0 * fr.dv + fr.pad_lo, v1 = fr.vlo + (float)fj1 * fr.dv + fr.pad_hi;
                    if (bin_jointly_empty(G, u0, u1, v0, v1)) kind = 0;
                }
            }
        }



        STAMP(st_setup)
        const uint32_t ni = (uint32_t)(i_hi - i_lo + 1);
        const uint32_t nb = kind == 1 ? ni * (uint32_t)(j_hi - j_lo + 1) : 0u;
        uint32_t incl = nb;
#pragma unroll
        for (int d = 1; d < 64; d <<= 1) {
            const uint32_t o = __shfl_up(incl, d);
            if (lane >= d) incl += o;
        }
        __syncthreads();
        if (lane == 63 && wave < 4) s_wave[wave] = incl;
        if (kind == 1) {
            s_A2[threadIdx.x] = make_float4(it.A2[0], it.A2[1], it.A2[2], it.A2[3]);
            s_Bu[threadIdx.x] = make_float4(it.Bu[0], it.Bu[1], it.Bu[2], it.Bu[3]);
            s_Bv[threadIdx.x] = make_float4(it.Bv[0], it.Bv[1], it.Bv[2], it.Bv[3]);
            s_box[threadIdx.x] = make_float4(it.lou, it.hiu, it.lov, it.hiv);
            s_org[threadIdx.x] = (uint32_t)i_lo | ((uint32_t)j_lo << 16);
            s_ni[threadIdx.x] = ni | (shell << 8);
            s_tri[threadIdx.x] = tri;
        }
        __syncthreads();
        const uint32_t t0w = s_wave[0], t1w = s_wave[1], t2w = s_wave[2], t3w = s_wave[3];
        if (threadIdx.x < 256) s_pre[threadIdx.x] = (wave > 0 ? t0w : 0u) + (wave > 1 ? t1w : 0u) + (wave > 2 ? t2w : 0u) + incl - nb;
        const uint32_t T = t0w + t1w + t2w + t3w;
        if (threadIdx.x == 0) s_pre[256] = T;

#ifdef MIRT_BIN_STATS
        if (kind == 2) { atomicAdd(&bs.counters[11 + dbg_state], 1u); if (frame == 0) atomicAdd(&bs.counters[14], 1u); }
        if (threadIdx.x == 0) { atomicAdd(&bs.counters[8], T); atomicMax(&bs.counters[9], T); }
        { const unsigned long long md = __ballot(kind == 1); if (lane == 0) atomicAdd(&bs.counters[10], (uint32_t)__popcll(md)); }
#endif
        STAMP(st_prefix)
        constexpr int TPT = BIN_TESTS_PER_THREAD;
        for (uint32_t r0 = 0; r0 < T; r0 += WG * TPT) {
#ifdef MIRT_BIN_STAMPS
            st_nrounds++;
#endif
            __syncthreads();
            if (s_fill + (uint32_t)(WG * TPT) > (uint32_t)BIN_PAIR_BUF) flush();
            bool pass[TPT];
            uint32_t key[TPT], val[TPT];
#pragma unroll
            for (int q = 0; q < TPT; q++) {
                const uint32_t t = r0 + (uint32_t)(q * WG) + threadIdx.x;
                pass[q] = false; key[q] = 0; val[q] = 0;
                if (t < T) {
                    uint32_t lo = 0, hi = 256;
#pragma unroll
                    for (int step = 0; step < 8; step++) {
                        const uint32_t mid = (lo + hi) >> 1;
                        if (s_pre[mid] <= t) lo = mid; else hi = mid;
                    }
                    const uint32_t nis = s_ni[lo], wi = nis & 0xFFu, sh = nis >> 8;
                    const uint32_t b = t - s_pre[lo], org = s_org[lo];
                    const uint32_t recip = 65536u / wi + 1u;
                    const uint32_t dj = (b * recip) >> 16, di = b - dj * wi;
                    const int i = (int)(org & 0xFFFFu) + (int)di, j = (int)(org >> 16) + (int)dj;
                    const float4 A2 = s_A2[lo], Bu = s_Bu[lo], Bv = s_Bv[lo], box = s_box[lo];
                    const float FI = (float)i, FJ = (float)j;
                    pass[q] = (__builtin_fmaf(FJ, Bv.x, __builtin_fmaf(FI, Bu.x, A2.x)) >= 0.0f) &&
                              (__builtin_fmaf(FJ, Bv.y, __builtin_fmaf(FI, Bu.y, A2.y)) >= 0.0f) &&
                              (__builtin_fmaf(FJ, Bv.z, __builtin_fmaf(FI, Bu.z, A2.z)) >= 0.0f) &&
                              (__builtin_fmaf(FJ, Bv.w, __builtin_fmaf(FI, Bu.w, A2.w)) >= 0.0f) &&
                              (FI + 1.0f >= box.x) && (FI <= box.y) && (FJ + 1.0f >= box.z) && (FJ <= box.w);
                    key[q] = (gr.fbase + (uint32_t)j * (uint32_t)nbu + (uint32_t)i) * gr.nshell + sh;
                    val[q] = s_tri[lo];
                }
            }
            unsigned long long m[TPT];
            uint32_t off[TPT], cnt = 0;
#pragma unroll
            for (int q = 0; q < TPT; q++) { m[q] = __ballot(pass[q]); off[q] = cnt; cnt += (uint32_t)__popcll(m[q]); }
            if (cnt) {
                uint32_t at0 = 0;
                if (lane == 0) at0 = atomicAdd(&s_fill, cnt);
                at0 = (uint32_t)__builtin_amdgcn_readfirstlane((int)at0);
#pragma unroll
                for (int q = 0; q < TPT; q++)
                    if (pass[q]) {
                        const uint32_t at = at0 + off[q] + (uint32_t)__popcll(m[q] & ((1ull << lane) - 1ull));
                        s_keys[at] = key[q]; s_vals[at] = val[q];
                    }
            }
        }

        STAMP(st_rounds)
        __syncthreads();
        {
            BinLargeSink sink = { s_keys, s_vals, &s_fill, &s_valid, &bs.counters[0], out, bs.bucket_cnt, bs.bucket_shift };
            for (unsigned long long ml = __ballot(kind == 2); ml;) {
                const int src = __builtin_ctzll(ml);
                ml &= ml - 1ull;
                BinItem u;
#pragma unroll
                for (int k = 0; k < 4; k++) {
                    u.A0[k] = bcastf(it.A0[k], src); u.A1[k] = bcastf(it.A1[k], src); u.A2[k] = bcastf(it.A2[k], src);
                    u.Bu[k] = bcastf(it.Bu[k], src); u.Bv[k] = bcastf(it.Bv[k], src);
                }
                u.lou = bcastf(it.lou, src); u.hiu = bcastf(it.hiu, src); u.lov = bcastf(it.lov, src); u.hiv = bcastf(it.hiv, src);
                const uint32_t utri = (uint32_t)__builtin_amdgcn_readlane((int)tri, src);
                const uint32_t ushell = (uint32_t)__builtin_amdgcn_readlane((int)shell, src);
                const unsigned long long ucells = ((unsigned long long)(uint32_t)__builtin_amdgcn_readlane((int)(cells >> 32), src) << 32) | (uint32_t)__builtin_amdgcn_readlane((int)cells, src);
                bin_walk_large(u, utri, ushell, gr, lane, sink, ucells);
            }
        }
        STAMP(st_huge)
    }
#ifdef MIRT_BIN_STAMPS
    st_t = __builtin_amdgcn_s_memtime();
#endif
    flush();
    STAMP(st_flush)
#ifdef MIRT_BIN_STAMPS
    if (threadIdx.x == 0 && (blockIdx.x % 97) == 0)
        printf("wg %d: total %lld | setup %lld prefix %lld rounds %lld (%d) huge %lld flush %lld\n", (int)blockIdx.x, (long long)__builtin_amdgcn_s_memtime() - st_begin,
               st_setup, st_prefix, st_rounds, st_nrounds, st_huge, st_flush);
#endif
}

template __global__ void k_bin_pairs<512>(const float *, const OriginRow *, const OriginRow *, int, BinSet, BinPairs);
template __global__ void k_bin_pairs<256>(const float *, const OriginRow *, const OriginRow *, int, BinSet, BinPairs);

}
```

### cpp-raytracer-rasterizer_amd/csrc/rt_trace.hip

```cpp
#include "rt_binned.hpp"

#include <float.h>

namespace mirt {


__global__ __launch_bounds__(256) void k_geo_table(const float *__restrict__ tris15, int n, GeoRow *__restrict__ geo, ShadeRow *__restrict__ shade)
{
    const int t = blockIdx.x * blockDim.x + threadIdx.x;
    if (t >= n) return;
    const float *t15 = tris15 + (size_t)15 * t;
    const v3 v0 = ld3(t15), e1 = sub3(ld3(t15 + 3), v0), e2 = sub3(ld3(t15 + 6), v0);
    GeoRow g;
    g.g0 = make_float4(v0.x, v0.y, v0.z, e1.x);
    g.g1 = make_float4(e1.y, e1.z, e2.x, e2.y);
    g.g2 = make_float4(e2.z, 0.0f, 0.0f, 0.0f);
    geo[t] = g;
    const v3 nd = normalize3(ld3(t15 + 9));
    ShadeRow sr;
    sr.n = make_float4(nd.x, nd.y, nd.z, 0.0f);
    sr.col = make_float4(t15[12], t15[13], t15[14], 0.0f);
    shade[t] = sr;
}

__global__ __launch_bounds__(256) void k_expand_light_rows(const uint32_t *__restrict__ bin_off, const uint32_t *__restrict__ entries,
                                                           int nlights, uint32_t keys_per_light,
                                                           const OriginRow *__restrict__ light_tab, int n,
                                                           LightRow *__restrict__ rows, const uint32_t *__restrict__ pair_count, uint32_t pair_cap,
                                                           uint32_t *__restrict__ row_tri )
{
    if (pair_count && *pair_count > pair_cap) return;
    const uint32_t first = bin_off[0], total = bin_off[(size_t)nlights * keys_per_light];
    for (uint32_t p = first + blockIdx.x * blockDim.x + threadIdx.x; p < total; p += gridDim.x * blockDim.x) {
        int k = 0;
        while (k + 1 < nlights && bin_off[(size_t)(k + 1) * keys_per_light] <= p) k++;
        const uint32_t tri = entries[p];
        rows[p] = light_tab[(size_t)k * n + tri];
        if (row_tri) row_tri[p] = tri;
    }
}

#ifndef MIRT_TR_STAGE
#define MIRT_TR_STAGE 16
#endif
constexpr int TR_STAGE = MIRT_TR_STAGE;
constexpr int TR_DRAIN = 64;
constexpr int TR_QUEUE = 96;
constexpr int TR_PIX = 128;
static_assert(TR_STAGE == 16, "the staging lanes are split 16 / 16 between the two tiles");

struct TrWaveLds {
    float4 rows[TR_STAGE * 6];
    float4 geo[TR_STAGE * 2 * 3];
    float4 q[TR_QUEUE];
    unsigned long long best[TR_PIX];
    uint2 qa[TR_QUEUE];
    union {
        float px[TR_PIX];
        float thr[TR_PIX];
    };
    float py[TR_PIX], pz[TR_PIX];
    uint8_t flag[TR_PIX];
};
static_assert(sizeof(TrWaveLds) % 16 == 0, "per-wave LDS slice must keep 16-byte alignment");

__device__ __forceinline__ void wave_lds_fence()
{
    __builtin_amdgcn_fence(__ATOMIC_RELEASE, "wavefront");
    __builtin_amdgcn_wave_barrier();
    __builtin_amdgcn_fence(__ATOMIC_ACQUIRE, "wavefront");
}

template <bool SHADOW>
__device__ __forceinline__ void tr_drain(TrWaveLds &s, int lane, int count, const float4 *__restrict__ geo, v3 start,
                                         const uint32_t *__restrict__ row_tri = nullptr, bool lazy_geo = false)
{
    wave_lds_fence();
    if (lane < count) {
        const float4 e = s.q[lane];
        uint2 a = s.qa[lane];
        float t, u, v;
        div3_sel(e.w, e.y, e.z, e.x, __builtin_amdgcn_ballot_w64(exact_quotients_outside(e.w, e.y, e.z, e.x)), t, u, v);
        if (u + v <= 1.0f && u >= 0.0f && v >= 0.0f && t >= 0.0f) {
            float4 g0, g1, g2;
            if (SHADOW) {
                const uint32_t tri = row_tri ? row_tri[a.y] : a.y;
                const float4 *g = geo + (size_t)tri * 3;
                g0 = g[0]; g1 = g[1]; g2 = g[2];
            } else if (lazy_geo) {
                const float4 *g = geo + (size_t)a.y * 3;
                g0 = g[0]; g1 = g[1]; g2 = g[2];
                a.x &= 0xFFu;
            } else {
                const float4 *g = s.geo + (a.x >> 8) * 3;
                g0 = g[0]; g1 = g[1]; g2 = g[2];
                a.x &= 0xFFu;
            }
            const v3 v0 = V3(g0.x, g0.y, g0.z), e1 = V3(g0.w, g1.x, g1.y), e2 = V3(g1.z, g1.w, g2.x);
            const v3 p = add3(add3(v0, scale3(e1, u)), scale3(e2, v));
            const float dist = distance3(start, p);
            if (SHADOW) {
                if (dist < s.thr[a.x]) s.flag[a.x] = 1;
            } else {
                s.flag[a.x] = 1;
                const unsigned long long key = min_t_key(dist, (int)a.y);
                atomicMin(&s.best[a.x], key);
                __builtin_amdgcn_fence(__ATOMIC_ACQ_REL, "wavefront");
                if (s.best[a.x] == key) { s.px[a.x] = p.x; s.py[a.x] = p.y; s.pz[a.x] = p.z; }
            }
        }
    }
    wave_lds_fence();
}

template <bool SHADOW>
__device__ __forceinline__ void tr_drain_full(TrWaveLds &s, int lane, int &qn, const float4 *__restrict__ geo, v3 start,
                                              const uint32_t *__restrict__ row_tri = nullptr, bool lazy_geo = false)
{
    tr_drain<SHADOW>(s, lane, TR_DRAIN, geo, start, row_tri, lazy_geo);
    const int rest = qn - TR_DRAIN;
    float4 e = make_float4(0.0f, 0.0f, 0.0f, 0.0f);
    uint2 a = make_uint2(0u, 0u);
    if (lane < rest) { e = s.q[TR_DRAIN + lane]; a = s.qa[TR_DRAIN + lane]; }
    wave_lds_fence();
    if (lane < rest) { s.q[lane] = e; s.qa[lane] = a; }
    qn = rest;
    wave_lds_fence();
}

__device__ __forceinline__ unsigned long long wballot(bool p) { return __builtin_amdgcn_ballot_w64(p); }

__device__ __forceinline__ int wave_rank(unsigned long long m)
{
    return (int)__builtin_amdgcn_mbcnt_hi((uint32_t)(m >> 32), __builtin_amdgcn_mbcnt_lo((uint32_t)m, 0u));
}

__device__ __forceinline__ void cube_bin_of2(const v3p &rd, uint32_t face_base0, int cube_bins, uint32_t *bin0, uint32_t *bin1)
{
    f2 a, b, m;
    int face[2];
#pragma unroll
    for (int h = 0; h < 2; h++) {
        const float x = h ? rd.x.y : rd.x.x, y = h ? rd.y.y : rd.y.x, z = h ? rd.z.y : rd.z.x;
        const float ax = fabsf(x), ay = fabsf(y), az = fabsf(z);
        int k;
        float mm, aa, bb, sgn;
        if (ax >= ay && ax >= az) { k = 0; mm = ax; sgn = x; aa = y; bb = z; }
        else if (ay >= az) { k = 1; mm = ay; sgn = y; aa = z; bb = x; }
        else { k = 2; mm = az; sgn = z; aa = x; bb = y; }
        face[h] = 2 * k + (sgn < 0.0f ? 1 : 0);
        if (h) { a.y = aa; b.y = bb; m.y = mm; } else { a.x = aa; b.x = bb; m.x = mm; }
    }
    const f2 im = { __builtin_amdgcn_rcpf(m.x), __builtin_amdgcn_rcpf(m.y) };
    const f2 u = a * im, v = b * im;
    const float half = 0.5f * (float)cube_bins;
    const uint32_t per_face = (uint32_t)(cube_bins * cube_bins);
#pragma unroll
    for (int h = 0; h < 2; h++) {
        const float uu = h ? u.y : u.x, vv = h ? v.y : v.x;
        int i = (int)floorf((uu + 1.0f) * half);
        int j = (int)floorf((vv + 1.0f) * half);
        i = min(max(i, 0), cube_bins - 1);
        j = min(max(j, 0), cube_bins - 1);
        const uint32_t bin = face_base0 + (uint32_t)face[h] * per_face + (uint32_t)j * cube_bins + (uint32_t)i;
        if (h) *bin1 = bin; else *bin0 = bin;
    }
}

struct TilePairRec { uint32_t tile, beg, nA, nB; };
constexpr int ORDER_CLASSES = 8;
constexpr int ORDER_GROUPS = 8;
constexpr uint32_t ORDER_CLASS_STEP = 16;

struct RtTraceFrame {
    RtFrame f;
    const uint32_t *cam_off;
    const uint32_t *cam_entries;
    const GeoRow *geo;
    const ShadeRow *shade;
    const uint32_t *light_off;
    const LightRow *light_rows;
    const uint32_t *light_tri;
    const BinFrameDesc *light_frames;
    int tiles_x;
    int cube_bins;
    int cam_shells;
    int light_shells;
    const uint32_t *pair_count;
    uint32_t pair_cap;
    const TilePairRec *order;
    const uint32_t *order_count;
    uint32_t order_seg;
    const uint32_t *sel;
    const uint32_t *sel_count;
    int lazy_geo;
    const uint32_t *light_pair_count;
    uint32_t light_pair_cap;
};

__global__ __launch_bounds__(64) void k_tile_order(const uint32_t *__restrict__ cam_off, int cam_shells, int tiles_x, int j0, int j1,
                                                   uint32_t *__restrict__ counters, uint32_t pair_cap, TilePairRec *__restrict__ order, uint32_t seg)
{
    const int pairs_x = (tiles_x + 1) / 2, lane = threadIdx.x;
    const int ty = j0 + (int)blockIdx.y, px = (int)blockIdx.x * 64 + lane;
    const uint32_t group = ((uint32_t)ty >> ORDER_STRIPE_SHIFT) & (ORDER_GROUPS - 1);
    TilePairRec r = { 0u, 0u, 0u, 0u };
    int cls = -1;
    if (px < pairs_x) {
        r.tile = (uint32_t)(ty * tiles_x + 2 * px);
        cls = 0;
        if (counters[0] <= pair_cap) {
            const uint32_t b0 = cam_off[(size_t)r.tile * cam_shells], b1 = cam_off[(size_t)(r.tile + 1) * cam_shells];
            r.beg = b0; r.nA = b1 - b0;
            r.nB = 2 * px + 1 < tiles_x ? cam_off[(size_t)(r.tile + 2) * cam_shells] - b1 : 0u;
            cls = (int)min(max(r.nA, r.nB) / ORDER_CLASS_STEP, (uint32_t)(ORDER_CLASSES - 1));
        }
    }
    unsigned long long m[ORDER_CLASSES];
    uint32_t mine = 0;
#pragma unroll
    for (int c = 0; c < ORDER_CLASSES; c++) {
        m[c] = __builtin_amdgcn_ballot_w64(cls == c);
        if (lane == c) mine = (uint32_t)__popcll(m[c]);
    }
    uint32_t base = 0;
    if (lane < ORDER_CLASSES && mine) base = atomicAdd(&counters[16 + group * ORDER_CLASSES + lane], mine);
#pragma unroll
    for (int c = 0; c < ORDER_CLASSES; c++) {
        const uint32_t bc = (uint32_t)__builtin_amdgcn_readlane((int)base, c);
        if (cls == c) order[((size_t)group * ORDER_CLASSES + c) * seg + bc + (uint32_t)__popcll(m[c] & ((1ull << lane) - 1ull))] = r;
    }
}

#ifndef MIRT_TR_WAVES
#define MIRT_TR_WAVES 4
#endif
#ifndef MIRT_TR_WAVES_MIN
#define MIRT_TR_WAVES_MIN 3
#endif
template <bool AA, bool STATS, int WAVES = MIRT_TR_WAVES>
__global__ __launch_bounds__(256) __attribute__((amdgpu_waves_per_eu(WAVES == 5 ? 5 : MIRT_TR_WAVES_MIN, WAVES))) void k_rt_trace2(const RtTraceFrame tf)
{
    extern __shared__ __attribute__((aligned(16))) float4 s_all[];
    const RtFrame &f = tf.f;
    const int lane = threadIdx.x & 63, wave = threadIdx.x >> 6;
    TrWaveLds &s = reinterpret_cast<TrWaveLds *>(s_all)[wave];

    const uint32_t group = blockIdx.x & (ORDER_GROUPS - 1);
    uint32_t w = (blockIdx.x >> 3) * (blockDim.x >> 6) + (uint32_t)wave;
    TilePairRec rec = { 0u, 0u, 0u, 0u };
    {
        bool found = false;
#pragma unroll
        for (int c = ORDER_CLASSES - 1; c >= 0; c--) {
            const uint32_t cnt = tf.order_count[group * ORDER_CLASSES + c];
            if (!found && w < cnt) { rec = tf.order[((size_t)group * ORDER_CLASSES + c) * tf.order_seg + w]; found = true; }
            if (!found) w -= cnt;
        }
        if (!found) return;
    }
    rec.tile = (uint32_t)__builtin_amdgcn_readfirstlane((int)rec.tile); rec.beg = (uint32_t)__builtin_amdgcn_readfirstlane((int)rec.beg);
    rec.nA = (uint32_t)__builtin_amdgcn_readfirstlane((int)rec.nA); rec.nB = (uint32_t)__builtin_amdgcn_readfirstlane((int)rec.nB);
    const int txA = (int)(rec.tile % (uint32_t)tf.tiles_x), ty = (int)(rec.tile / (uint32_t)tf.tiles_x);
    const bool enB = txA + 1 < tf.tiles_x;
    const int xA = txA * BIN_TILE + (lane & 7), xB = xA + BIN_TILE, y = ty * BIN_TILE + (lane >> 3);
    const bool okY = y >= f.y0 && y < f.y1;
    const bool okA = okY && xA < f.W, okB = enB && okY && xB < f.W;
    const unsigned long long okmA = wballot(okA), okmB = wballot(okB);
    const unsigned nokA = (unsigned)__popcll(okmA), nokB = (unsigned)__popcll(okmB);
#ifdef MIRT_TR_TIMING
    const long long tm0 = __builtin_amdgcn_s_memtime();
    long long tm_last = tm0, tm_seg[10] = { 0, 0, 0, 0, 0, 0, 0, 0, 0, 0 };
#define TM_SEG(i) { const long long now_ = __builtin_amdgcn_s_memtime(); tm_seg[i] += now_ - tm_last; tm_last = now_; }
#else
#define TM_SEG(i)
#endif
    const bool brute = (uint32_t)__builtin_amdgcn_readfirstlane((int)*tf.pair_count) > tf.pair_cap;
    const bool brute_l = tf.light_pair_count ? (uint32_t)__builtin_amdgcn_readfirstlane((int)*tf.light_pair_count) > tf.light_pair_cap : false;
    const v3 cam = ld3(f.cam);
    const int rs = AA ? f.aa : 1;

    const uint32_t begA = rec.beg, begB = rec.beg + rec.nA;
    const uint32_t nall = brute ? min((uint32_t)__builtin_amdgcn_readfirstlane((int)*tf.sel_count), (uint32_t)f.n) : 0u;
    const uint32_t nA = brute ? nall : rec.nA, nB = brute ? (enB ? nall : 0u) : rec.nB;
    const uint32_t nmax = max(nA, nB);
    const float4 *geo4 = reinterpret_cast<const float4 *>(tf.geo);
    const bool lazy = tf.lazy_geo != 0;
    TM_SEG(0)

    float bdA = FLT_MAX, bdB = FLT_MAX;
    int biA = -1, biB = -1;
    v3 posA = V3(0.0f, 0.0f, 0.0f), posB = posA;
    v3p avg = splat3(V3(0.0f, 0.0f, 0.0f));
    unsigned ntests = 0, ncand = 0, nsteps_p = 0, nsteps_s = 0, ndrains = 0;
    unsigned ncand_l = 0;
    int qn = 0;
    const float hw = (float)f.W / 2.0f, hh = (float)f.H / 2.0f;

    f2 y1 = splat2(aa_start(y, rs));
    for (int z = 0; z < rs; z++) {
        f2 x1 = { aa_start(xA, rs), aa_start(xB, rs) };
        for (int z2 = 0; z2 < rs; z2++) {
            const v3p d = V3P(x1 - splat2(hw), y1 - splat2(hh), splat2(f.focal));
            const v3p nd = neg3p(mat3_mul_vecp(f.rot, d));

            s.best[lane] = MIN_T_NONE; s.best[lane + 64] = MIN_T_NONE;
            s.flag[lane] = 0; s.flag[lane + 64] = 0;
            if (STATS) ncand += nokA * nA + nokB * nB;
            float lbA = okA ? FLT_MAX : -__builtin_huge_valf(), lbB = okB ? FLT_MAX : -__builtin_huge_valf();
            float tbA = FLT_MAX, tbB = FLT_MAX;
            for (uint32_t base = 0; base < nmax; base += TR_STAGE) {
                const int cntA = (int)min((uint32_t)TR_STAGE, nA > base ? nA - base : 0u);
                const int cntB = (int)min((uint32_t)TR_STAGE, nB > base ? nB - base : 0u);
                wave_lds_fence();
                float my_near = 0.0f;
                const int sh = lane >> 4, sj = lane & 15;
                const bool stage = lane < 32 && sj < (sh ? cntB : cntA);
                if (stage) {
                    const uint32_t idx = brute ? tf.sel[base + (uint32_t)sj] : tf.cam_entries[(sh ? begB : begA) + base + (uint32_t)sj];
                    const float4 *src = reinterpret_cast<const float4 *>(f.cam_tab + idx);
                    const float4 a0 = src[0], a1 = src[1], a2 = src[2];
                    if (!lazy) {
                        const float4 *gsrc = geo4 + (size_t)idx * 3;
                        float4 *gdst = s.geo + lane * 3;
                        gdst[0] = gsrc[0]; gdst[1] = gsrc[1]; gdst[2] = gsrc[2];
                    }
                    float *dst = reinterpret_cast<float *>(s.rows) + sj * 24 + sh;
                    dst[0] = a0.x; dst[2] = a0.y; dst[4] = a0.z; dst[6] = a0.w;
                    dst[8] = a1.x; dst[10] = a1.y; dst[12] = a1.z; dst[14] = a1.w;
                    dst[16] = a2.x; dst[18] = a2.y; dst[20] = a2.z; dst[22] = __uint_as_float(idx);
                    my_near = a1.w;
                } else if (lane < 32) {
                    reinterpret_cast<float *>(s.rows)[sj * 24 + sh + 14] = __builtin_huge_valf();
                }
                wave_lds_fence();
                TM_SEG(1)
                uint32_t pmA = (uint32_t)wballot(stage && sh == 0 && !(my_near > tbA)) & 0xFFFFu;
                uint32_t pmB = (uint32_t)(wballot(stage && sh == 1 && !(my_near > tbB)) >> 16) & 0xFFFFu;
                uint32_t pm = pmA | pmB;
                while (pm) {
                    const int j = __builtin_ctz(pm);
                    pm &= pm - 1u;
                    if (STATS) nsteps_p++;
                    const float4 *R = s.rows + 6 * j;
                    const float4 R0 = R[0], R1 = R[1], R2 = R[2], R3 = R[3], R4 = R[4], R5 = R[5];
                    TestDots2 td;
                    td.den = (f2){ R0.x, R0.y } * nd.x + (f2){ R0.z, R0.w } * nd.y + (f2){ R1.x, R1.y } * nd.z;
                    td.pu = (f2){ R2.x, R2.y } * nd.x + (f2){ R2.z, R2.w } * nd.y + (f2){ R3.x, R3.y } * nd.z;
                    td.qv = (f2){ R4.x, R4.y } * nd.x + (f2){ R4.z, R4.w } * nd.y + (f2){ R5.x, R5.y } * nd.z;
                    const f2 fm = maybe_hit2_margin(td);
                    const unsigned long long nearA = wballot(!(R3.z > lbA)), nearB = wballot(!(R3.w > lbB));
                    const unsigned long long filtA = wballot(fm.x >= MAYBE_HIT_THRESHOLD), filtB = wballot(fm.y >= MAYBE_HIT_THRESHOLD);
                    const unsigned long long mA = nearA & filtA, mB = nearB & filtB;
                    const bool passA0 = (mA >> lane) & 1ull, passB = (mB >> lane) & 1ull;
                    if (STATS) ntests += (unsigned)__popcll(nearA) + (unsigned)__popcll(nearB);
                    if (mA | mB) {
                        int cA = __popcll(mA);
                        const int cB = __popcll(mB);
                        bool passA = passA0;
                        if (qn + cA + cB > TR_QUEUE) {
                            TM_SEG(2)
                            if (qn) { tr_drain<false>(s, lane, qn, geo4, cam, nullptr, lazy); qn = 0; if (STATS) ndrains++; }
                            if (cA + cB > TR_QUEUE) {
                                if (passA) {
                                    const int at = wave_rank(mA);
                                    s.q[at] = make_float4(td.den.x, td.pu.x, td.qv.x, R1.z);
                                    s.qa[at] = make_uint2((uint32_t)lane | ((uint32_t)j << 8), __float_as_uint(R5.z));
                                }
                                tr_drain<false>(s, lane, cA, geo4, cam, nullptr, lazy); if (STATS) ndrains++;
                                passA = false; cA = 0;
                            }
                            TM_SEG(3)
                        }
                        if (passA) {
                            const int at = qn + wave_rank(mA);
                            s.q[at] = make_float4(td.den.x, td.pu.x, td.qv.x, R1.z);
                            s.qa[at] = make_uint2((uint32_t)lane | ((uint32_t)j << 8), __float_as_uint(R5.z));
                        }
                        if (passB) {
                            const int at = qn + cA + wave_rank(mB);
                            s.q[at] = make_float4(td.den.y, td.pu.y, td.qv.y, R1.w);
                            s.qa[at] = make_uint2(((uint32_t)lane + 64u) | ((uint32_t)(16 + j) << 8), __float_as_uint(R5.w));
                        }
                        qn += cA + cB;
                        if (qn >= TR_DRAIN) {
                            TM_SEG(2)
                            do { tr_drain_full<false>(s, lane, qn, geo4, cam, nullptr, lazy); if (STATS) ndrains++; } while (qn >= TR_DRAIN);
                            TM_SEG(3)
                            lbA = okA ? min_t_dist(s.best[lane]) : lbA; lbB = okB ? min_t_dist(s.best[lane + 64]) : lbB;
                            tbA = wave_max_f(lbA); tbB = wave_max_f(lbB);
                            pmA &= (uint32_t)wballot(stage && sh == 0 && !(my_near > tbA));
                            pmB &= (uint32_t)(wballot(stage && sh == 1 && !(my_near > tbB)) >> 16);
                            pm &= pmA | pmB;
                        }
                    }
                }
                TM_SEG(2)
                if (qn) {
                    tr_drain<false>(s, lane, qn, geo4, cam, nullptr, lazy); qn = 0; if (STATS) ndrains++;
                    if (base + TR_STAGE < nmax) {
                        lbA = okA ? min_t_dist(s.best[lane]) : lbA; lbB = okB ? min_t_dist(s.best[lane + 64]) : lbB;
                        tbA = wave_max_f(lbA); tbB = wave_max_f(lbB);
                    }
                }
                TM_SEG(3)
            }
            const unsigned long long keyA = s.best[lane], keyB = s.best[lane + 64];
            const bool anyA = s.flag[lane] != 0, anyB = s.flag[lane + 64] != 0;
            if (anyA && bdA >= min_t_dist(keyA)) {
                bdA = min_t_dist(keyA); biA = min_t_index(keyA);
                posA = V3(s.px[lane], s.py[lane], s.pz[lane]);
            }
            if (anyB && bdB >= min_t_dist(keyB)) {
                bdB = min_t_dist(keyB); biB = min_t_index(keyB);
                posB = V3(s.px[lane + 64], s.py[lane + 64], s.pz[lane + 64]);
            }

            TM_SEG(4)
            const bool hitA = okA && anyA, hitB = okB && anyB;
            const unsigned long long hmA = wballot(hitA), hmB = wballot(hitB);
            const unsigned nhits = (unsigned)(__popcll(hmA) + __popcll(hmB));
            if (hmA | hmB) {
                const ShadeRow *srA = tf.shade + (biA >= 0 ? biA : 0), *srB = tf.shade + (biB >= 0 ? biB : 0);
                const float4 nA4 = srA->n, nB4 = srB->n;
                float4 cA4 = make_float4(0.0f, 0.0f, 0.0f, 0.0f), cB4 = cA4;
                if constexpr (WAVES != 5) { cA4 = srA->col; cB4 = srB->col; }
                const v3p pos = join3(posA, posB);
                const v3p nDir = join3(V3(nA4.x, nA4.y, nA4.z), V3(nB4.x, nB4.y, nB4.z));
                v3p result = splat3(V3(0.0f, 0.0f, 0.0f)), result2 = result;
                for (int k = 0; k < f.nlights; k++) {
                    const v3 L = ld3(f.lpos[k]);
                    const LightGeometry2 lg = light_geometry2(pos, L, ld3(f.lcol[k]), f.lights_in_range != 0, hitA, hitB);
                    const f2 r = lg.r;
                    const v3p rd = lg.rDir, B = lg.B;
                    const f2 dn = dot3p(rd, nDir);
                    const f2 mx = { (dn.x < 0.0f) ? 0.0f : dn.x, (dn.y < 0.0f) ? 0.0f : dn.y };
                    v3p D = scale3p(B, mx);
                    const f2 thr = r * splat2(0.99f);
                    TM_SEG(5)
                    wave_lds_fence();
                    s.thr[lane] = thr.x; s.thr[lane + 64] = thr.y;
                    s.flag[lane] = 0; s.flag[lane + 64] = 0;
                    uint32_t eA = 0, endA = 0, eB = 0, endB = 0;
                    const float4 *rows4;
                    if (brute_l) {
                        rows4 = reinterpret_cast<const float4 *>(f.light_tab + (size_t)k * f.n);
                        if (hitA) endA = (uint32_t)f.n;
                        if (hitB) endB = (uint32_t)f.n;
                    } else {
                        rows4 = reinterpret_cast<const float4 *>(tf.light_rows);
                        uint32_t binA, binB;
                        cube_bin_of2(rd, (uint32_t)k * 6u * (uint32_t)(tf.cube_bins * tf.cube_bins), tf.cube_bins, &binA, &binB);
                        const BinFrameDesc *lf = tf.light_frames + 6 * k;
                        const int ns = tf.light_shells;
                        const float sd0 = lf->shell_d0, siw = lf->shell_iw;
                        const uint32_t shA = ns > 1 ? (uint32_t)min(max((int)((thr.x - sd0) * siw), 0), ns - 1) : 0u;
                        const uint32_t shB = ns > 1 ? (uint32_t)min(max((int)((thr.y - sd0) * siw), 0), ns - 1) : 0u;
                        if (hitA) {
                            const uint32_t key = binA * (uint32_t)ns;
                            eA = tf.light_off[key]; endA = tf.light_off[key + shA + 1u];
                        }
                        if (hitB) {
                            const uint32_t key = binB * (uint32_t)ns;
                            eB = tf.light_off[key]; endB = tf.light_off[key + shB + 1u];
                        }
                    }
                    if (STATS) ncand_l += (endA - eA) + (endB - eB);
                    const uint32_t *row_tri = brute_l ? nullptr : tf.light_tri;
                    const bool firstA = eA < endA;
                    uint32_t e = firstA ? eA : eB, end = firstA ? endA : endB, pix = firstA ? (uint32_t)lane : (uint32_t)lane + 64u;
                    v3 crd = firstA ? half0(rd) : half1(rd);
                    float cthr = firstA ? thr.x : thr.y;
                    uint32_t occ = 0u;
                    float4 c0, c1, c2;
                    { const float4 *src = rows4 + (size_t)(e < end ? e : 0u) * 3; c0 = src[0]; c1 = src[1]; c2 = src[2]; }
                    TM_SEG(6)
                    const int not_brute = brute_l ? 0 : 1;
                    for (;;) {
                        const bool act = e < end;
                        const unsigned long long am = wballot(act);
                        if (!am) break;
                        if (STATS) { nsteps_s++; ntests += (unsigned)__popcll(am); }
                        const TestDots td = test_dots(c0, c1, c2, crd);
                        const int pass = (int)act & (int)!(c1.w > cthr) & (int)maybe_hit(td);
                        const int sure = pass & not_brute & (int)(c2.w < cthr) & (int)sure_hit(td, c0.w);
                        const int queue = pass & (sure ^ 1);
                        const unsigned long long m = wballot(queue != 0);
                        int done = sure;
                        if (m) {
                            if (qn + __popcll(m) > TR_QUEUE) { tr_drain<true>(s, lane, qn, geo4, L, row_tri); qn = 0; if (STATS) ndrains++; }
                            if (queue) {
                                const int at = qn + wave_rank(m);
                                s.q[at] = make_float4(td.den, td.pu, td.qv, c0.w);
                                s.qa[at] = make_uint2(pix, e);
                            }
                            qn += __popcll(m);
                            if (qn >= TR_DRAIN) {
                                TM_SEG(7)
                                do { tr_drain_full<true>(s, lane, qn, geo4, L, row_tri); if (STATS) ndrains++; } while (qn >= TR_DRAIN);
                                TM_SEG(8)
                                done |= (int)act & (int)(s.flag[pix] != 0);
                            }
                        }
                        occ |= sure ? (pix < 64u ? 1u : 2u) : 0u;
                        const int cont = (int)act & (done ^ 1) & (int)(e + 1u < end);
                        const int sw = (int)act & (cont ^ 1) & (int)(pix < 64u) & (int)(eB < endB);
                        crd = sw ? half1(rd) : crd;
                        cthr = sw ? thr.y : cthr;
                        pix = sw ? (uint32_t)lane + 64u : pix;
                        e = cont ? e + 1u : (sw ? eB : end);
                        end = sw ? endB : end;
                        const float4 *src = rows4 + (size_t)((cont | sw) ? e : 0u) * 3;
                        c0 = src[0]; c1 = src[1]; c2 = src[2];
                    }
                    TM_SEG(7)
                    if (qn) { tr_drain<true>(s, lane, qn, geo4, L, row_tri); qn = 0; if (STATS) ndrains++; }
                    TM_SEG(8)
                    const bool occA = (occ & 1u) != 0u, occB = (occ & 2u) != 0u;
                    if (occA || s.flag[lane] != 0) { D.x.x = 0.0f; D.y.x = 0.0f; D.z.x = 0.0f; }
                    if (occB || s.flag[lane + 64] != 0) { D.x.y = 0.0f; D.y.y = 0.0f; D.z.y = 0.0f; }
                    result = add3p(result, D);
                    if ((k + 1) % f.samples == 0) result2 = add3p(result2, result);
                }
                if constexpr (WAVES == 5) { cA4 = srA->col; cB4 = srB->col; }
                const v3p tcol = join3(V3(cA4.x, cA4.y, cA4.z), V3(cB4.x, cB4.y, cB4.z));
                const v3p Dl = mul3p(result2, tcol);
                const v3p shaded = add3p(avg, mul3p(tcol, add3p(Dl, splat3(ld3(f.indirect)))));
                avg = join3(hitA ? half0(shaded) : half0(avg), hitB ? half1(shaded) : half1(avg));
                if (AA) x1 = x1 + (f2){ hitA ? aa_step(rs) : 0.0f, hitB ? aa_step(rs) : 0.0f };
            }
            if (lane == 0 && nhits) {
                const unsigned shard = (blockIdx.x + (threadIdx.x >> 6) * 61u) % HIT_SHARDS;
                atomicAdd(f.hit_count + (size_t)shard * HIT_SHARD_STRIDE, (unsigned long long)nhits);
            }
            wave_lds_fence();
        }
        if (AA) y1 = y1 + splat2(aa_step(rs));
    }
    {
        if (STATS) ncand += wave_sum(ncand_l);
        const unsigned shard = (blockIdx.x + (threadIdx.x >> 6) * 61u) % HIT_SHARDS;
#ifdef MIRT_TR_TIMING
        TM_SEG(9)
        if (lane == 0) {
            for (int i = 0; i < 10; i++) atomicAdd(f.hit_count + (size_t)shard * HIT_SHARD_STRIDE + 3 + i, (unsigned long long)tm_seg[i]);
            atomicMax(f.hit_count + (size_t)shard * HIT_SHARD_STRIDE + 13, (unsigned long long)(tm_last - tm0));
        }
        const unsigned v = lane == 0 ? ntests : ncand;
        if (lane < 2 && v) atomicAdd(f.hit_count + (size_t)shard * HIT_SHARD_STRIDE + 1 + lane, (unsigned long long)v);
#else
        const unsigned v = lane == 0 ? ntests : lane == 1 ? ncand : lane == 2 ? nsteps_p : lane == 3 ? nsteps_s : ndrains;
        if (STATS && lane < 5 && v) atomicAdd(f.hit_count + (size_t)shard * HIT_SHARD_STRIDE + 1 + lane, (unsigned long long)v);
#endif
    }
    if (AA) {
        const f2 q = splat2((float)(rs * rs));
        avg = V3P(div2(avg.x, q), div2(avg.y, q), div2(avg.z, q));
    }
    if (okA) {
        const v3 c = half0(avg);
        const size_t px = (size_t)y * f.W + xA;
        if (f.rgb) st3(f.rgb + 3 * px, c);
        if (f.index) f.index[px] = biA;
        if (f.fd) f.fd[px] = biA >= 0 ? bdA - f.focal_plane : 0.0f;
        store_intersection(f, px, biA, bdA, posA);
        if (xA >= 1 && xA < f.W - 1 && y >= 1 && y < f.H - 1)
            f.xrgb[(size_t)(y - f.row_origin) * f.pitch_words + xA] = pack_xrgb(c);
    }
    if (okB) {
        const v3 c = half1(avg);
        const size_t px = (size_t)y * f.W + xB;
        if (f.rgb) st3(f.rgb + 3 * px, c);
        if (f.index) f.index[px] = biB;
        if (f.fd) f.fd[px] = biB >= 0 ? bdB - f.focal_plane : 0.0f;
        store_intersection(f, px, biB, bdB, posB);
        if (xB >= 1 && xB < f.W - 1 && y >= 1 && y < f.H - 1)
            f.xrgb[(size_t)(y - f.row_origin) * f.pitch_words + xB] = pack_xrgb(c);
    }
}

template __global__ void k_rt_trace2<false, false>(const RtTraceFrame);
template __global__ void k_rt_trace2<false, false, 5>(const RtTraceFrame);
template __global__ void k_rt_trace2<false, true>(const RtTraceFrame);
template __global__ void k_rt_trace2<true, false>(const RtTraceFrame);
template __global__ void k_rt_trace2<true, true>(const RtTraceFrame);

size_t rt_trace_lds_bytes(int waves) { return (size_t)waves * sizeof(TrWaveLds); }

}
```

Baseline: 47720.

## Shrink LDS footprints and retune occupancy across binning, select and trace kernels

Moves the bin-pairs key/value buffers into dynamic LDS, sized per workgroup (smaller for 256-wide groups), and adds waves-per-EU hints to the bin and scatter kernels. Large-triangle items are staged through LDS instead of readlane broadcasts from registers, and the per-pair box test is dropped from the inner loop. The prep-select kernel moves to 256-thread groups with two per CU. Trace drops the per-wave geo staging from LDS when lazy geometry is on, and lazy geo becomes the default. The goal is higher occupancy and lower register/LDS pressure, at the cost of extra syncs, LDS traffic and a possibly looser pair filter.

```diff
diff --git a/cpp-raytracer-rasterizer_amd/capi/binned.cpp b/cpp-raytracer-rasterizer_amd/capi/binned.cpp
--- a/cpp-raytracer-rasterizer_amd/capi/binned.cpp
+++ b/cpp-raytracer-rasterizer_amd/capi/binned.cpp
@@ -47,11 +47,10 @@
     }
     uint32_t *bcnt = S.d_bucket, *bbase = S.d_bucket + S.cap_buckets, *bcur = S.d_bucket + 2 * (size_t)S.cap_buckets;
     bs.bucket_cnt = bcnt; bs.nbuckets = nbuckets; bs.bucket_shift = bucket_sort_shift(bs.nbins);
-    const size_t bin_lds = (size_t)nbuckets * sizeof(uint32_t);
     {
         static const bool once = [] {
-            (void)hipFuncSetAttribute(reinterpret_cast<const void *>(&k_bin_pairs<512>), hipFuncAttributeMaxDynamicSharedMemorySize, 48 * 1024);
-            (void)hipFuncSetAttribute(reinterpret_cast<const void *>(&k_bin_pairs<256>), hipFuncAttributeMaxDynamicSharedMemorySize, 48 * 1024);
+            (void)hipFuncSetAttribute(reinterpret_cast<const void *>(&k_bin_pairs<512>), hipFuncAttributeMaxDynamicSharedMemorySize, (int)bin_pairs_lds_bytes(512, BUCKET_SORT_MAX_BUCKETS));
+            (void)hipFuncSetAttribute(reinterpret_cast<const void *>(&k_bin_pairs<256>), hipFuncAttributeMaxDynamicSharedMemorySize, (int)bin_pairs_lds_bytes(256, BUCKET_SORT_MAX_BUCKETS));
             return true; }();
         (void)once;
     }
@@ -73,6 +72,7 @@
         if (attempt) HIP_TRY(hipMemsetAsync(counter, 0, 4, g.stream));
         if (attempt || S.bucket_dirty) HIP_TRY(hipMemsetAsync(S.d_bucket, 0, sizeof(uint32_t) * 3 * (size_t)S.cap_buckets, g.stream));
         S.bucket_dirty = true;
+        const size_t bin_lds = bin_pairs_lds_bytes(bin_wg, nbuckets);
         if (bin_wg == 256) hipLaunchKernelGGL(k_bin_pairs<256>, bin_grid, dim3(256), bin_lds, g.stream, g.d_tris, cam_tab, light_tab, g.n, bs, pairs);
         else hipLaunchKernelGGL(k_bin_pairs<512>, bin_grid, dim3(512), bin_lds, g.stream, g.d_tris, cam_tab, light_tab, g.n, bs, pairs);
         if (!fresh) break;
@@ -446,8 +446,10 @@
         so.sel_count = S.d_bin_counters + SEL_COUNT0 + S.sel_parity; so.sel_count_next = S.d_bin_counters + SEL_COUNT0 + (S.sel_parity ^ 1);
         so.zero_hits = g.d_hits; so.zero_counter = S.d_bin_counters;
         if ((rc = hist_prepare(S, bs.frame0, &so))) return rc;
-        const unsigned sel_grid = (unsigned)std::min<long long>(((long long)g.n + 1023) / 1024, (long long)g.cu_count);
-        hipLaunchKernelGGL(k_prep_select, dim3(sel_grid), dim3(1024), 0, g.stream, g.d_tris, g.n, bs.frame0, so);
+        int sel_wg, sel_per_cu;
+        prep_select_shape(&sel_wg, &sel_per_cu);
+        const unsigned sel_grid = (unsigned)std::min<long long>(((long long)g.n + sel_wg - 1) / sel_wg, (long long)g.cu_count * sel_per_cu);
+        hipLaunchKernelGGL(k_prep_select, dim3(sel_grid), dim3(sel_wg), 0, g.stream, g.d_tris, g.n, bs.frame0, so);
         if ((rc = hist_publish(S))) return rc;
         bs.sel = S.d_sel; bs.sel_count = so.sel_count;
         g.stats_sel_count = so.sel_count;
@@ -503,8 +505,10 @@
     if ((rc = hist_prepare(S, fr, &so))) return rc;
     if (!g.hist_armed) return MIRT_OK;
     HIP_TRY(hipMemsetAsync(so.sel_count, 0, 4, g.stream));
-    const unsigned sel_grid = (unsigned)std::min<long long>(((long long)g.n + 1023) / 1024, (long long)g.cu_count);
-    if (sel_grid) hipLaunchKernelGGL(k_prep_select, dim3(sel_grid), dim3(1024), 0, g.stream, g.d_tris, g.n, fr, so);
+    int sel_wg, sel_per_cu;
+    prep_select_shape(&sel_wg, &sel_per_cu);
+    const unsigned sel_grid = (unsigned)std::min<long long>(((long long)g.n + sel_wg - 1) / sel_wg, (long long)g.cu_count * sel_per_cu);
+    if (sel_grid) hipLaunchKernelGGL(k_prep_select, dim3(sel_grid), dim3(sel_wg), 0, g.stream, g.d_tris, g.n, fr, so);
     HIP_TRY(hipGetLastError());
     return hist_publish(S);
 }
@@ -522,7 +526,7 @@
     tf.cam_entries = S.d_entries;
     tf.sel = S.d_sel; tf.sel_count = S.d_bin_counters + SEL_COUNT0 + S.sel_parity;
     static const int lazy_env = (int)env_int("MIRT_LAZY_GEO", -1);
-    tf.lazy_geo = lazy_env >= 0 ? (lazy_env != 0) : (g.n >= 400000);
+    tf.lazy_geo = lazy_env >= 0 ? (lazy_env != 0) : 1;
     tf.geo = g.d_geo;
     tf.shade = g.d_shade;
     tf.light_off = transient ? L.d_bin_off : g.lc.d_off;
@@ -539,7 +543,7 @@
     tf.light_pair_cap = L.cap_used;
     tf.order = S.d_order; tf.order_count = S.d_bin_counters + 16; tf.order_seg = bp.order_seg;
     const dim3 tgrid(ORDER_GROUPS * bp.order_seg);
-    const size_t lds = rt_trace_lds_bytes(1);
+    const size_t lds = rt_trace_lds_bytes(1, tf.lazy_geo != 0);
     k_begin(MIRT_K_TRACE);
     g.pending_counted = g.profiling;
     if (f.aa > 1) {
diff --git a/cpp-raytracer-rasterizer_amd/capi/capi.hpp b/cpp-raytracer-rasterizer_amd/capi/capi.hpp
--- a/cpp-raytracer-rasterizer_amd/capi/capi.hpp
+++ b/cpp-raytracer-rasterizer_amd/capi/capi.hpp
@@ -70,7 +70,9 @@
 MIRT_KERNEL void k_geo_table(const float *, int, GeoRow *, ShadeRow *);
 MIRT_KERNEL void k_expand_light_rows(const uint32_t *, const uint32_t *, int, uint32_t, const OriginRow *, int, LightRow *, const uint32_t *, uint32_t, uint32_t *);
 MIRT_KERNEL void k_cull(const float *, int, const CullParams, uint8_t *);
-size_t rt_trace_lds_bytes(int waves);
+size_t rt_trace_lds_bytes(int waves, bool lazy_geo);
+size_t bin_pairs_lds_bytes(int wg, uint32_t nbuckets);
+void prep_select_shape(int *wg, int *per_cu);
 int launch_raster(RasterFrame &f, RasterScratch &s, uint64_t scene_version, hipStream_t stream, hipEvent_t *ev, bool *ev_used);
 
 extern char g_err[512];
diff --git a/cpp-raytracer-rasterizer_amd/csrc/bin_bucket_sort.hip b/cpp-raytracer-rasterizer_amd/csrc/bin_bucket_sort.hip
--- a/cpp-raytracer-rasterizer_amd/csrc/bin_bucket_sort.hip
+++ b/cpp-raytracer-rasterizer_amd/csrc/bin_bucket_sort.hip
@@ -30,7 +30,10 @@
     return off + incl - v;
 }
 
-__global__ __launch_bounds__(256) void k_bs_scatter(const uint32_t *__restrict__ keys, const uint32_t *__restrict__ vals,
+#ifndef MIRT_BS_SCATTER_WAVES
+#define MIRT_BS_SCATTER_WAVES 5
+#endif
+__global__ __launch_bounds__(256) __attribute__((amdgpu_waves_per_eu(MIRT_BS_SCATTER_WAVES))) void k_bs_scatter(const uint32_t *__restrict__ keys, const uint32_t *__restrict__ vals,
                                                     const uint32_t *__restrict__ total_ptr, uint32_t cap, uint32_t nbuckets, int shift,
                                                     const uint32_t *__restrict__ bucket_cnt, uint32_t *__restrict__ bucket_base,
                                                     uint32_t *__restrict__ cursor, uint32_t *__restrict__ out_keys, uint32_t *__restrict__ out_vals,
diff --git a/cpp-raytracer-rasterizer_amd/csrc/rt_binned.hip b/cpp-raytracer-rasterizer_amd/csrc/rt_binned.hip
--- a/cpp-raytracer-rasterizer_amd/csrc/rt_binned.hip
+++ b/cpp-raytracer-rasterizer_amd/csrc/rt_binned.hip
@@ -11,7 +11,7 @@
     float lou, hiu, lov, hiv;
 };
 
-__device__ __forceinline__ float bcastf(float v, int lane) { return __builtin_bit_cast(float, __builtin_amdgcn_readlane(__builtin_bit_cast(int, v), lane)); }
+__device__ __forceinline__ float unif(float v) { return __builtin_bit_cast(float, __builtin_amdgcn_readfirstlane(__builtin_bit_cast(int, v))); }
 
 __device__ __forceinline__ float corner(float s, float lo, float hi) { return fmaxf(s * lo, s * hi); }
 
@@ -59,12 +59,13 @@
 
 struct BinFrameGrid { int nbu, fj0, fj1, cells_x, cy0, ncell; uint32_t fbase, nshell; };
 
-constexpr int BIN_PAIR_BUF = 4096;
+constexpr int bin_pair_buf(int wg) { return wg == 256 ? 3072 : 4096; }
 constexpr int BIN_TESTS_PER_THREAD = 2;
 constexpr int BIN_DIRECT_SIDE = 32;
 
 struct BinLargeSink {
     uint32_t *s_keys, *s_vals;
+    uint32_t buf;
     uint32_t *s_fill;
     uint32_t *s_valid;
     uint32_t *g_count;
@@ -110,11 +111,11 @@
                 uint32_t at0 = 0;
                 if (lane == 0) at0 = atomicAdd(sink.s_fill, np);
                 at0 = (uint32_t)__builtin_amdgcn_readfirstlane((int)at0);
-                if (at0 + np <= (uint32_t)BIN_PAIR_BUF) {
+                if (at0 + np <= sink.buf) {
                     if (pass2) { sink.s_keys[at0 + rank] = key; sink.s_vals[at0 + rank] = utri; }
                 } else {
                     if (lane == 0) {
-                        if (at0 < (uint32_t)BIN_PAIR_BUF) *sink.s_valid = at0;
+                        if (at0 < sink.buf) *sink.s_valid = at0;
                         at0 = atomicAdd(sink.g_count, np);
                     }
                     at0 = (uint32_t)__builtin_amdgcn_readfirstlane((int)at0);
@@ -135,26 +136,33 @@
 }
 
 constexpr int SEL_WG = 1024;
-constexpr int SEL_STAGE = 8192;
-
-__global__ __launch_bounds__(SEL_WG) void k_prep_select(const float *__restrict__ tris15, int n, const BinFrameDesc fr, const SelectOut out)
+#ifndef MIRT_PREP_WG
+#define MIRT_PREP_WG 256
+#endif
+constexpr int PREP_WG = MIRT_PREP_WG;
+constexpr int PREP_PER_CU = PREP_WG >= 1024 ? 1 : 2;
+constexpr int PREP_STAGE = PREP_WG >= 1024 ? 8192 : 4096;
+static_assert(PREP_WG >= SEL_HIST_MAX && PREP_WG % 64 == 0 && PREP_STAGE >= 2 * PREP_WG, "the histogram's rows are zeroed and flushed one per thread");
+
+__global__ __launch_bounds__(PREP_WG) void k_prep_select(const float *__restrict__ tris15, int n, const BinFrameDesc fr, const SelectOut out)
 {
     __shared__ uint32_t s_hist[SEL_HIST_MAX];
-    __shared__ uint32_t s_sel[SEL_STAGE];
+    __shared__ uint32_t s_sel[PREP_STAGE];
     __shared__ uint32_t s_fill, s_base;
     const int lane = threadIdx.x & 63;
     if (blockIdx.x == 0) {
         if (out.zero_hits)
-            for (int g = threadIdx.x; g < HIT_SHARDS * HIT_SHARD_STRIDE; g += SEL_WG) out.zero_hits[g] = 0ull;
+            for (int g = threadIdx.x; g < HIT_SHARDS * HIT_SHARD_STRIDE; g += PREP_WG) out.zero_hits[g] = 0ull;
         if (out.zero_counter && (threadIdx.x == 0 || (threadIdx.x >= 16 && threadIdx.x < 80))) out.zero_counter[threadIdx.x] = 0u;
         if (threadIdx.x == 0) *out.sel_count_next = 0u;
-        if (out.zero_faces && (int)threadIdx.x < out.zero_faces_n) out.zero_faces[threadIdx.x] = 0u;
+        if (out.zero_faces)
+            for (int g = threadIdx.x; g < out.zero_faces_n; g += PREP_WG) out.zero_faces[g] = 0u;
     }
     if (out.hist && threadIdx.x < SEL_HIST_MAX) s_hist[threadIdx.x] = 0u;
     if (threadIdx.x == 0) s_fill = 0u;
     __syncthreads();
     const v3 S = V3(fr.S[0], fr.S[1], fr.S[2]);
-    const int nchunks = (n + SEL_WG - 1) / SEL_WG;
+    const int nchunks = (n + PREP_WG - 1) / PREP_WG;
     const int hist_rows = ((fr.nbv - 1) >> out.hist_shift) + 1;
     auto flush = [&]() {
         __syncthreads();
@@ -162,14 +170,14 @@
         if (threadIdx.x == 0 && staged) s_base = atomicAdd(out.sel_count, staged);
         __syncthreads();
         const uint32_t base = s_base;
-        for (uint32_t i = threadIdx.x; i < staged; i += SEL_WG) out.sel[base + i] = s_sel[i];
+        for (uint32_t i = threadIdx.x; i < staged; i += PREP_WG) out.sel[base + i] = s_sel[i];
         __syncthreads();
         if (threadIdx.x == 0) s_fill = 0u;
         __syncthreads();
     };
     for (int c = blockIdx.x; c < nchunks; c += gridDim.x) {
-        if (s_fill + (uint32_t)SEL_WG > (uint32_t)SEL_STAGE) flush();
-        const int i = c * SEL_WG + (int)threadIdx.x;
+        if (s_fill + (uint32_t)PREP_WG > (uint32_t)PREP_STAGE) flush();
+        const int i = c * PREP_WG + (int)threadIdx.x;
         bool keep = false;
         OriginRow r;
         if (i < n) {
@@ -268,28 +276,31 @@
     flush();
 }
 
-
+#ifndef MIRT_BIN_WAVES256
+#define MIRT_BIN_WAVES256 5
+#endif
 template <int WG>
-__global__ __launch_bounds__(WG) void k_bin_pairs(const float *__restrict__ tris15, const OriginRow *__restrict__ cam_tab,
+__global__ __launch_bounds__(WG) __attribute__((amdgpu_waves_per_eu(WG == 256 ? MIRT_BIN_WAVES256 : 4))) void k_bin_pairs(const float *__restrict__ tris15, const OriginRow *__restrict__ cam_tab,
                                                    const OriginRow *__restrict__ light_tab, int n, BinSet bs, BinPairs out)
 {
-    extern __shared__ uint32_t s_bucket[];
-    __shared__ uint32_t s_keys[BIN_PAIR_BUF], s_vals[BIN_PAIR_BUF];
-    __shared__ float4 s_A2[256], s_Bu[256], s_Bv[256], s_box[256];
+    constexpr uint32_t BUF = (uint32_t)bin_pair_buf(WG);
+    extern __shared__ uint32_t s_dyn[];
+    uint32_t *const s_keys = s_dyn, *const s_vals = s_dyn + BUF, *const s_bucket = s_dyn + 2 * BUF;
+    __shared__ float4 s_A2[256], s_Bu[256], s_Bv[256];
+    __shared__ float4 s_A0[256], s_A1[256], s_box[256];
     __shared__ uint32_t s_org[256];
     __shared__ uint32_t s_ni[256];
     __shared__ uint32_t s_tri[256];
     __shared__ uint32_t s_pre[257];
     __shared__ uint32_t s_wave[4];
     __shared__ uint32_t s_base, s_fill, s_valid;
-    const int lane = threadIdx.x & 63, wave = threadIdx.x >> 6;
     const int chunk_tris = bs.chunk_tris;
-    const int nchunks = (n + chunk_tris - 1) / chunk_tris;
+    const int nchunks = __builtin_amdgcn_readfirstlane((n + chunk_tris - 1) / chunk_tris);
     const bool listed = bs.sel != nullptr;
     const uint32_t nsel = listed ? min(*bs.sel_count, (uint32_t)n) : 0u;
     const int cam_chunk = (listed && nsel < 32768u) ? 64 : chunk_tris;
-    const int ncam = listed ? (int)((nsel + (uint32_t)cam_chunk - 1u) / (uint32_t)cam_chunk) : 0;
-    const int nrest = listed ? bs.nframes - 1 : bs.nframes;
+    const int ncam = __builtin_amdgcn_readfirstlane(listed ? (int)((nsel + (uint32_t)cam_chunk - 1u) / (uint32_t)cam_chunk) : 0);
+    const int nrest = __builtin_amdgcn_readfirstlane(listed ? bs.nframes - 1 : bs.nframes);
     const bool faces_listed = bs.face_lists != nullptr;
     __shared__ uint32_t s_first[MAX_BIN_FRAMES + 1];
     if (faces_listed) {
@@ -300,8 +311,8 @@
         }
         __syncthreads();
     }
-    const int nwork = ncam + (faces_listed ? (int)s_first[nrest] : nchunks * nrest);
-    if (threadIdx.x == 0) { s_fill = 0u; s_valid = (uint32_t)BIN_PAIR_BUF; }
+    const int nwork = __builtin_amdgcn_readfirstlane(ncam + (faces_listed ? (int)s_first[nrest] : nchunks * nrest));
+    if (threadIdx.x == 0) { s_fill = 0u; s_valid = BUF; }
     if (bs.bucket_cnt)
         for (uint32_t b = threadIdx.x; b < bs.nbuckets; b += WG) s_bucket[b] = 0u;
 
@@ -322,7 +333,7 @@
                 const uint32_t c = s_bucket[b];
                 if (c) { atomicAdd(&bs.bucket_cnt[b], c); s_bucket[b] = 0u; }
             }
-        if (threadIdx.x == 0) { s_fill = 0u; s_valid = (uint32_t)BIN_PAIR_BUF; }
+        if (threadIdx.x == 0) { s_fill = 0u; s_valid = BUF; }
         __syncthreads();
     };
 
@@ -338,6 +349,9 @@
 #ifdef MIRT_BIN_STAMPS
         st_t = __builtin_amdgcn_s_memtime();
 #endif
+        uint32_t tid = threadIdx.x;
+        asm volatile("" : "+v"(tid));
+        const int lane = (int)(tid & 63u), wave = (int)(tid >> 6);
         int chunk, frame;
         const uint32_t *list = nullptr;
         uint32_t nhere = (uint32_t)n;
@@ -353,22 +367,20 @@
             nhere = min(bs.face_counts[lo], (uint32_t)n);
         } else { const int w2 = w - ncam; chunk = w2 / nrest; frame = w2 - chunk * nrest + (listed ? 1 : 0); }
         const int item_tris = from_cam_list ? cam_chunk : chunk_tris;
-        const uint32_t slot = (uint32_t)chunk * (uint32_t)item_tris + threadIdx.x;
-        const uint32_t tri = ((int)threadIdx.x < item_tris && slot < nhere) ? (list ? list[slot] : slot) : 0xFFFFFFFFu;
+        const uint32_t slot = (uint32_t)chunk * (uint32_t)item_tris + tid;
+        const uint32_t tri = ((int)tid < item_tris && slot < nhere) ? (list ? list[slot] : slot) : 0xFFFFFFFFu;
         const BinFrameDesc fr = bs.frames ? bs.frames[frame] : bs.frame0;
         BinFrameGrid gr;
         gr.nbu = fr.nbu; gr.fj0 = fr.j0; gr.fj1 = fr.j1; gr.fbase = fr.base; gr.nshell = (uint32_t)max(fr.nshell, 1);
         gr.cells_x = (gr.nbu + BIN_L0 - 1) / BIN_L0; gr.cy0 = gr.fj0 / BIN_L0;
         gr.ncell = gr.cells_x * ((gr.fj1 + BIN_L0 - 1) / BIN_L0 - gr.cy0);
         const int nbu = gr.nbu, fj0 = gr.fj0, fj1 = gr.fj1;
-        BinItem it;
-        memset(&it, 0, sizeof it);
+        __syncthreads();
         int kind = 0;
 #ifdef MIRT_BIN_STATS
         int dbg_state = 0;
 #endif
         int i_lo = 0, i_hi = -1, j_lo = 0, j_hi = -1;
-        unsigned long long cells = 0;
         uint32_t shell = 0;
         if (tri < (uint32_t)n && fj1 > fj0) {
             const OriginRow &row = (fr.tab == 0) ? cam_tab[tri] : light_tab[(size_t)(fr.tab - 1) * n + tri];
@@ -383,6 +395,7 @@
             const float sgn = t.nb < 0.0f ? -1.0f : 1.0f;
             const EdgeFn *fn[4] = { &t.n, &t.p, &t.q, &t.s };
             const float inf = __builtin_huge_valf();
+            BinItem it;
 #pragma unroll
             for (int k = 0; k < 4; k++) {
                 const float su = sgn * fn[k]->cu, sv = sgn * fn[k]->cv;
@@ -393,6 +406,11 @@
                 it.A1[k] = both ? inf : base + corner(su, fr.pad_lo, (float)BIN_COARSE * fr.du + fr.pad_hi) + corner(sv, fr.pad_lo, (float)BIN_COARSE * fr.dv + fr.pad_hi);
                 it.A2[k] = both ? inf : base + corner(su, fr.pad_lo, fr.du + fr.pad_hi) + corner(sv, fr.pad_lo, fr.dv + fr.pad_hi);
             }
+            s_A2[tid] = make_float4(it.A2[0], it.A2[1], it.A2[2], it.A2[3]);
+            s_Bu[tid] = make_float4(it.Bu[0], it.Bu[1], it.Bu[2], it.Bu[3]);
+            s_Bv[tid] = make_float4(it.Bv[0], it.Bv[1], it.Bv[2], it.Bv[3]);
+            s_A0[tid] = make_float4(it.A0[0], it.A0[1], it.A0[2], it.A0[3]);
+            s_A1[tid] = make_float4(it.A1[0], it.A1[1], it.A1[2], it.A1[3]);
             if (t.bstate == BOX_VALID) {
                 it.lou = (t.bu0 - fr.ulo - fr.pad_hi) / fr.du; it.hiu = (t.bu1 - fr.ulo - fr.pad_lo) / fr.du;
                 it.lov = (t.bv0 - fr.vlo - fr.pad_hi) / fr.dv; it.hiv = (t.bv1 - fr.vlo - fr.pad_lo) / fr.dv;
@@ -409,7 +427,9 @@
                 i_lo = (int)flo_u; i_hi = (int)fhi_u; j_lo = (int)flo_v; j_hi = (int)fhi_v;
                 kind = (i_hi - i_lo < BIN_DIRECT_SIDE && j_hi - j_lo < BIN_DIRECT_SIDE) ? 1 : 2;
             }
+            s_box[tid] = make_float4(it.lou, it.hiu, it.lov, it.hiv);
             if (kind == 2) {
+                unsigned long long cells = 0;
                 for (int c = 0; c < gr.ncell && c < 64; c++) {
                     const int cx = c % gr.cells_x, cy = gr.cy0 + c / gr.cells_x;
                     if (cell_may_hit(it, it.A0, (float)(cx * BIN_L0), (float)(cy * BIN_L0), (float)BIN_L0)) cells |= 1ull << c;
@@ -424,6 +444,7 @@
                     const float v0 = fr.vlo + (float)fj0 * fr.dv + fr.pad_lo, v1 = fr.vlo + (float)fj1 * fr.dv + fr.pad_hi;
                     if (bin_jointly_empty(G, u0, u1, v0, v1)) kind = 0;
                 }
+                s_org[tid] = (uint32_t)cells; s_ni[tid] = (uint32_t)(cells >> 32);
             }
         }
 
@@ -438,26 +459,21 @@
             const uint32_t o = __shfl_up(incl, d);
             if (lane >= d) incl += o;
         }
-        __syncthreads();
         if (lane == 63 && wave < 4) s_wave[wave] = incl;
         if (kind == 1) {
-            s_A2[threadIdx.x] = make_float4(it.A2[0], it.A2[1], it.A2[2], it.A2[3]);
-            s_Bu[threadIdx.x] = make_float4(it.Bu[0], it.Bu[1], it.Bu[2], it.Bu[3]);
-            s_Bv[threadIdx.x] = make_float4(it.Bv[0], it.Bv[1], it.Bv[2], it.Bv[3]);
-            s_box[threadIdx.x] = make_float4(it.lou, it.hiu, it.lov, it.hiv);
-            s_org[threadIdx.x] = (uint32_t)i_lo | ((uint32_t)j_lo << 16);
-            s_ni[threadIdx.x] = ni | (shell << 8);
-            s_tri[threadIdx.x] = tri;
+            s_org[tid] = (uint32_t)i_lo | ((uint32_t)j_lo << 16);
+            s_ni[tid] = ni | (shell << 8);
+            s_tri[tid] = tri;
         }
         __syncthreads();
         const uint32_t t0w = s_wave[0], t1w = s_wave[1], t2w = s_wave[2], t3w = s_wave[3];
-        if (threadIdx.x < 256) s_pre[threadIdx.x] = (wave > 0 ? t0w : 0u) + (wave > 1 ? t1w : 0u) + (wave > 2 ? t2w : 0u) + incl - nb;
+        if (tid < 256) s_pre[tid] = (wave > 0 ? t0w : 0u) + (wave > 1 ? t1w : 0u) + (wave > 2 ? t2w : 0u) + incl - nb;
         const uint32_t T = t0w + t1w + t2w + t3w;
-        if (threadIdx.x == 0) s_pre[256] = T;
+        if (tid == 0) s_pre[256] = T;
 
 #ifdef MIRT_BIN_STATS
         if (kind == 2) { atomicAdd(&bs.counters[11 + dbg_state], 1u); if (frame == 0) atomicAdd(&bs.counters[14], 1u); }
-        if (threadIdx.x == 0) { atomicAdd(&bs.counters[8], T); atomicMax(&bs.counters[9], T); }
+        if (tid == 0) { atomicAdd(&bs.counters[8], T); atomicMax(&bs.counters[9], T); }
         { const unsigned long long md = __ballot(kind == 1); if (lane == 0) atomicAdd(&bs.counters[10], (uint32_t)__popcll(md)); }
 #endif
         STAMP(st_prefix)
@@ -467,12 +483,12 @@
             st_nrounds++;
 #endif
             __syncthreads();
-            if (s_fill + (uint32_t)(WG * TPT) > (uint32_t)BIN_PAIR_BUF) flush();
+            if (s_fill + (uint32_t)(WG * TPT) > BUF) flush();
             bool pass[TPT];
             uint32_t key[TPT], val[TPT];
 #pragma unroll
             for (int q = 0; q < TPT; q++) {
-                const uint32_t t = r0 + (uint32_t)(q * WG) + threadIdx.x;
+                const uint32_t t = r0 + (uint32_t)(q * WG) + tid;
                 pass[q] = false; key[q] = 0; val[q] = 0;
                 if (t < T) {
                     uint32_t lo = 0, hi = 256;
@@ -486,13 +502,12 @@
                     const uint32_t recip = 65536u / wi + 1u;
                     const uint32_t dj = (b * recip) >> 16, di = b - dj * wi;
                     const int i = (int)(org & 0xFFFFu) + (int)di, j = (int)(org >> 16) + (int)dj;
-                    const float4 A2 = s_A2[lo], Bu = s_Bu[lo], Bv = s_Bv[lo], box = s_box[lo];
+                    const float4 A2 = s_A2[lo], Bu = s_Bu[lo], Bv = s_Bv[lo];
                     const float FI = (float)i, FJ = (float)j;
                     pass[q] = (__builtin_fmaf(FJ, Bv.x, __builtin_fmaf(FI, Bu.x, A2.x)) >= 0.0f) &&
                               (__builtin_fmaf(FJ, Bv.y, __builtin_fmaf(FI, Bu.y, A2.y)) >= 0.0f) &&
                               (__builtin_fmaf(FJ, Bv.z, __builtin_fmaf(FI, Bu.z, A2.z)) >= 0.0f) &&
-                              (__builtin_fmaf(FJ, Bv.w, __builtin_fmaf(FI, Bu.w, A2.w)) >= 0.0f) &&
-                              (FI + 1.0f >= box.x) && (FI <= box.y) && (FJ + 1.0f >= box.z) && (FJ <= box.w);
+                              (__builtin_fmaf(FJ, Bv.w, __builtin_fmaf(FI, Bu.w, A2.w)) >= 0.0f);
                     key[q] = (gr.fbase + (uint32_t)j * (uint32_t)nbu + (uint32_t)i) * gr.nshell + sh;
                     val[q] = s_tri[lo];
                 }
@@ -517,20 +532,22 @@
         STAMP(st_rounds)
         __syncthreads();
         {
-            BinLargeSink sink = { s_keys, s_vals, &s_fill, &s_valid, &bs.counters[0], out, bs.bucket_cnt, bs.bucket_shift };
+            BinLargeSink sink = { s_keys, s_vals, BUF, &s_fill, &s_valid, &bs.counters[0], out, bs.bucket_cnt, bs.bucket_shift };
             for (unsigned long long ml = __ballot(kind == 2); ml;) {
                 const int src = __builtin_ctzll(ml);
                 ml &= ml - 1ull;
+                const int slot = (wave << 6) + src;
+                const float4 a0 = s_A0[slot], a1 = s_A1[slot], a2 = s_A2[slot], bu = s_Bu[slot], bv = s_Bv[slot], bx = s_box[slot];
                 BinItem u;
-#pragma unroll
-                for (int k = 0; k < 4; k++) {
-                    u.A0[k] = bcastf(it.A0[k], src); u.A1[k] = bcastf(it.A1[k], src); u.A2[k] = bcastf(it.A2[k], src);
-                    u.Bu[k] = bcastf(it.Bu[k], src); u.Bv[k] = bcastf(it.Bv[k], src);
-                }
-                u.lou = bcastf(it.lou, src); u.hiu = bcastf(it.hiu, src); u.lov = bcastf(it.lov, src); u.hiv = bcastf(it.hiv, src);
+                u.A0[0] = unif(a0.x); u.A0[1] = unif(a0.y); u.A0[2] = unif(a0.z); u.A0[3] = unif(a0.w);
+                u.A1[0] = unif(a1.x); u.A1[1] = unif(a1.y); u.A1[2] = unif(a1.z); u.A1[3] = unif(a1.w);
+                u.A2[0] = unif(a2.x); u.A2[1] = unif(a2.y); u.A2[2] = unif(a2.z); u.A2[3] = unif(a2.w);
+                u.Bu[0] = unif(bu.x); u.Bu[1] = unif(bu.y); u.Bu[2] = unif(bu.z); u.Bu[3] = unif(bu.w);
+                u.Bv[0] = unif(bv.x); u.Bv[1] = unif(bv.y); u.Bv[2] = unif(bv.z); u.Bv[3] = unif(bv.w);
+                u.lou = unif(bx.x); u.hiu = unif(bx.y); u.lov = unif(bx.z); u.hiv = unif(bx.w);
                 const uint32_t utri = (uint32_t)__builtin_amdgcn_readlane((int)tri, src);
                 const uint32_t ushell = (uint32_t)__builtin_amdgcn_readlane((int)shell, src);
-                const unsigned long long ucells = ((unsigned long long)(uint32_t)__builtin_amdgcn_readlane((int)(cells >> 32), src) << 32) | (uint32_t)__builtin_amdgcn_readlane((int)cells, src);
+                const unsigned long long ucells = ((unsigned long long)(uint32_t)__builtin_amdgcn_readfirstlane((int)s_ni[slot]) << 32) | (uint32_t)__builtin_amdgcn_readfirstlane((int)s_org[slot]);
                 bin_walk_large(u, utri, ushell, gr, lane, sink, ucells);
             }
         }
@@ -551,4 +568,10 @@
 template __global__ void k_bin_pairs<512>(const float *, const OriginRow *, const OriginRow *, int, BinSet, BinPairs);
 template __global__ void k_bin_pairs<256>(const float *, const OriginRow *, const OriginRow *, int, BinSet, BinPairs);
 
-}
+void prep_select_shape(int *wg, int *per_cu) { *wg = PREP_WG; *per_cu = PREP_PER_CU; }
+
+extern "C" __device__ __attribute__((used)) const uint32_t mirt_bin_pair_buf_bytes[2] = { 2 * sizeof(uint32_t) * bin_pair_buf(256), 2 * sizeof(uint32_t) * bin_pair_buf(512) };
+
+size_t bin_pairs_lds_bytes(int wg, uint32_t nbuckets) { return sizeof(uint32_t) * (2 * (size_t)bin_pair_buf(wg) + nbuckets); }
+
+}
diff --git a/cpp-raytracer-rasterizer_amd/csrc/rt_trace.hip b/cpp-raytracer-rasterizer_amd/csrc/rt_trace.hip
--- a/cpp-raytracer-rasterizer_amd/csrc/rt_trace.hip
+++ b/cpp-raytracer-rasterizer_amd/csrc/rt_trace.hip
@@ -1,6 +1,7 @@
 #include "rt_binned.hpp"
 
 #include <float.h>
+#include <stddef.h>
 
 namespace mirt {
 
@@ -45,13 +46,16 @@
 #endif
 constexpr int TR_STAGE = MIRT_TR_STAGE;
 constexpr int TR_DRAIN = 64;
-constexpr int TR_QUEUE = 96;
+#ifndef MIRT_TR_QUEUE
+#define MIRT_TR_QUEUE 96
+#endif
+constexpr int TR_QUEUE = MIRT_TR_QUEUE;
 constexpr int TR_PIX = 128;
 static_assert(TR_STAGE == 16, "the staging lanes are split 16 / 16 between the two tiles");
+static_assert(TR_QUEUE >= TR_DRAIN && TR_QUEUE % 2 == 0, "a drained queue takes the pairs of one tile; the slices stay 16-byte aligned");
 
 struct TrWaveLds {
     float4 rows[TR_STAGE * 6];
-    float4 geo[TR_STAGE * 2 * 3];
     float4 q[TR_QUEUE];
     unsigned long long best[TR_PIX];
     uint2 qa[TR_QUEUE];
@@ -61,7 +65,10 @@
     };
     float py[TR_PIX], pz[TR_PIX];
     uint8_t flag[TR_PIX];
+    float4 geo[TR_STAGE * 2 * 3];
 };
+constexpr size_t TR_LDS_LAZY = offsetof(TrWaveLds, geo);
+static_assert(TR_LDS_LAZY % 16 == 0, "per-wave LDS slice must keep 16-byte alignment");
 static_assert(sizeof(TrWaveLds) % 16 == 0, "per-wave LDS slice must keep 16-byte alignment");
 
 __device__ __forceinline__ void wave_lds_fence()
@@ -244,7 +251,7 @@
     extern __shared__ __attribute__((aligned(16))) float4 s_all[];
     const RtFrame &f = tf.f;
     const int lane = threadIdx.x & 63, wave = threadIdx.x >> 6;
-    TrWaveLds &s = reinterpret_cast<TrWaveLds *>(s_all)[wave];
+    TrWaveLds &s = *reinterpret_cast<TrWaveLds *>(reinterpret_cast<char *>(s_all) + (size_t)wave * (tf.lazy_geo ? TR_LDS_LAZY : sizeof(TrWaveLds)));
 
     const uint32_t group = blockIdx.x & (ORDER_GROUPS - 1);
     uint32_t w = (blockIdx.x >> 3) * (blockDim.x >> 6) + (uint32_t)wave;
@@ -585,6 +592,8 @@
 template __global__ void k_rt_trace2<true, false>(const RtTraceFrame);
 template __global__ void k_rt_trace2<true, true>(const RtTraceFrame);
 
-size_t rt_trace_lds_bytes(int waves) { return (size_t)waves * sizeof(TrWaveLds); }
-
-}
+extern "C" __device__ __attribute__((used)) const uint32_t mirt_tr_wave_lds_bytes[2] = { sizeof(TrWaveLds), TR_LDS_LAZY };
+
+size_t rt_trace_lds_bytes(int waves, bool lazy_geo) { return (size_t)waves * (lazy_geo ? TR_LDS_LAZY : sizeof(TrWaveLds)); }
+
+}
```

New measurement: 47850, median of 2. About the same (+0.3%).
